# mrazomej/BarBay.jl

Measured on AMD Instinct MI355X. Metric: ELBO-grad steps/sec, 50k barcodes x 8 timepoints, higher is better.
Workload: dtype f64

## Files before the change

barbay.jl_amd/csrc/bb_engine.hip:

```cpp
#include "../../include/barbay_hip.h"
#include "bb_block.h"
#include "bb_persist.h"
#include "bb_resident.h"
#include "bb_stream.h"
#include "bb_inst.h"
#include "bb_hier.h"
#include "bb_ppc.h"
#include "bb_freq.h"
#include "bb_score.h"
#include "bb_chain.h"
#include "bb_logp.h"
#include "bb_mathprobe.h"

#include <algorithm>
#include <cmath>
#include <cstdarg>
#include <cstdio>
#include <cstdlib>
#include <cstring>
#include <ctime>
#include <string>
#include <type_traits>
#include <vector>

static thread_local char g_err[512] = "";
static int bb_fail(int code, const char* fmt, ...) {
    va_list ap;
    va_start(ap, fmt);
    vsnprintf(g_err, sizeof g_err, fmt, ap);
    va_end(ap);
    return code;
}
extern "C" const char* bb_last_error(void) { return g_err; }

#include "bb_backend.h"

extern "C" const char* bb_version(void) { return BB_BACKEND_VERSION; }

#define BB_ENTER(h) DevGuard bb_dev_guard_((h)->o.device)

struct BBTuning {
    bool no_hist_pack, no_host_tables, no_res, no_persist, no_stream, force_stream, any_parity, force_allreduce, p2p_self;
    bool no_graph, graph_collective, no_regroup, no_reorder, nb_set, lead_set;
    int nb, res_nb, ng, lead, nthr, row_l2;
};

static BBTuning read_tuning() {
    auto set = [](const char* n) { return getenv(n) != nullptr; };
    auto num = [](const char* n, int unset) { const char* v = getenv(n); return v ? atoi(v) : unset; };
    auto on = [&](const char* n) { return num(n, 0) > 0; };
    BBTuning t{};
    t.no_hist_pack = on("BB_NO_HIST_PACK");
    t.no_host_tables = on("BB_NO_HOST_TABLES");
    t.no_res = on("BB_NO_RES");
    t.no_persist = on("BB_NO_PERSIST");
    t.no_stream = on("BB_NO_STREAM");
    t.force_stream = on("BB_TUNE_STREAM");
    t.any_parity = on("BB_TUNE_AP");
    t.force_allreduce = on("BB_FORCE_ALLREDUCE");
    t.p2p_self = on("BB_P2P_SELF");
    t.no_graph = set("BB_NO_GRAPH");
    t.graph_collective = set("BB_GRAPH_COLLECTIVE");
    t.no_regroup = set("BB_NO_REGROUP");
    t.no_reorder = set("BB_NO_REORDER");
    t.nb_set = set("BB_TUNE_NB");
    t.nb = num("BB_TUNE_NB", 0);
    t.res_nb = num("BB_TUNE_RES_NB", 0);
    t.ng = num("BB_TUNE_NG", 0);
    t.lead_set = set("BB_TUNE_LEAD");
    t.lead = num("BB_TUNE_LEAD", 65);
    if (t.lead < 10 || t.lead > 100) t.lead = 100;
    t.nthr = num("BB_TUNE_NTHR", 0) >= 64 ? num("BB_TUNE_NTHR", 0) / 64 * 64 : 0;
    t.row_l2 = num("BB_TUNE_ROW_L2", 1) == 0 ? 0 : 1;
    return t;
}

enum { IMPL_TWO_KERNEL = 0, IMPL_PERSIST = 1, IMPL_RES = 2, IMPL_STREAM = 3 };
struct LaunchPlan {
    int impl = IMPL_TWO_KERNEL;
    int P = 0;
    int NB = 0, NBL = 0, nblk = 0;
    int ng = 8, pf = 0;
    bool ms = false;
    const void* fn = nullptr;
    std::string name;
    const char* why = nullptr;
};

struct DevBuf {
    double* p = nullptr;
    size_t cap = 0;
    int grow(size_t n) {
        if (cap >= n) return 0;
        if (p) dfree(p);
        p = nullptr;
        cap = 0;
        void* q = nullptr;
        int rc = dmalloc(&q, n * 8);
        if (!rc) { p = (double*)q; cap = n; }
        return rc;
    }
};
enum {
    BUF_EPS,
    BUF_DBG,
    BUF_BANDS,
    BUF_LOGP,
    BUF_CHAIN,
    BUF_COUNT
};

struct bb_handle {
    DevModel M{};
    DevState S{};
    bb_advi_opts o{};
    std::vector<bb_block_range> blocks;
    std::vector<void*> owned;
    long long dev_bytes = 0;
    int NB = 0, nthr = 0, nblk = 0, ngeno_blk = 0;
    int tile_cap = 0;
    size_t lds_doubles = 0;
    size_t lds_doubles_p0 = 0;
    size_t lds_doubles_p = 0;
    long long b_lo = 0, b_hi = 0;
    int cus = 256;
    int g_lo = 0, g_hi = 0;
    std::vector<int> geno_ptr_h;
    long long* d_tile_b = nullptr;
    int* d_tile_g = nullptr;
    long long step = 0;
    int sample = 0;
    double elbo_const = 0.0;
    std::vector<double> ld_omega, ld_zero;
    void* p2p_inbox = nullptr;
    size_t p2p_rows_bytes = 0, p2p_bytes = 0, p2p_gran_off = 0;
    double* d_segtab = nullptr;
    int* d_ldstab = nullptr;
    size_t segtab_cap = 0, ldstab_cap = 0;
    void* p2p_peer[BB_MAX_WORLD] = {};
    bool p2p_ready = false, p2p_on = false;
    unsigned p2p_seq = 0;
    unsigned epoch0 = 0;
    long long req_steps = 0;
    bool p2p_first = false;
    unsigned* hstatus = nullptr;
    double* bak_mu = nullptr;
    double* bak_om = nullptr;
    DevBuf buf[BUF_COUNT];
    std::vector<double> logp_host;
    bbStream stream{};
    double last_run_ms = 0, avg_sample_ms = 0, avg_update_ms = 0;
    int launches_last_run = 0;
    int graph_launches = 0;
    int64_t bytes_sample = 0, bytes_update = 0;
    BackendState be;
    BBTuning tune{};
    LaunchPlan plan;
    BRLay Yh{};
    BRLay* dY = nullptr;
    DevModel* dM = nullptr;
    DevState* dS = nullptr;
    BBLds* dL = nullptr;
    BBLds Lp{};
    std::vector<bb_handle*> shards;
    bool group_resident = false;
    double* theta_buf = nullptr;
    bool theta_stale = false;
    bool in_group = false;
    std::vector<long long> cidx;
    std::vector<int> perm_m;
    bool use_reduce() const { return o.world_size > 1 || M.kind == BB_MODEL_GENOTYPE || tune.force_allreduce; }
};

template <class T>
static int dalloc(bb_handle* h, T** p, size_t count) {
    void* q = nullptr;
    int rc = dmalloc(&q, count * sizeof(T));
    if (rc) return rc;
    h->owned.push_back(q);
    h->dev_bytes += (long long)(count * sizeof(T));
    *p = (T*)q;
    return dzero(q, count * sizeof(T), h->stream);
}

extern "C" void bb_default_opts(bb_advi_opts* o) {
    memset(o, 0, sizeof *o);
    o->samples_per_step = 1;
    o->optimizer = BB_OPT_TRUNCATED_ADAGRAD;
    o->eta = 0.1;
    o->tau = 40.0;
    o->window = 100;
    o->resum_every = 0;
    o->pre = 1.0;
    o->post = 0.9;
    o->seed = 0;
    o->device = 0;
    o->rank = 0;
    o->world_size = 1;
    o->steps_per_graph = 0;
    o->elbo_every = 0;
    o->n_devices = 1;
    o->device_ids = nullptr;
}

static void add_block(bb_handle* h, const char* name, int kind, long long n, long long* off) {
    bb_block_range b;
    memset(&b, 0, sizeof b);
    snprintf(b.name, sizeof b.name, "%s", name);
    b.lo = *off;
    b.hi = *off + n;
    h->blocks.push_back(b);
    h->M.blk_lo[kind] = b.lo;
    h->M.blk_hi[kind] = b.hi;
    *off += n;
}

static int upload_prior(bb_handle* h, int kind, const bb_prior* p, double dmean, double dstd, const char* name,
                        bool vector_only, double* sum_log_std) {
    const long long n = h->M.blk_hi[kind] - h->M.blk_lo[kind];
    DevPrior& dp = h->M.pri[kind];
    dp.mean_e = nullptr;
    dp.inv_var_e = nullptr;
    if (!p || !p->mean || !p->std || p->n == 0) {
        dp.mean = dmean;
        dp.inv_var = 1.0 / (dstd * dstd);
        *sum_log_std += (double)n * log(dstd);
        return 0;
    }
    if (p->n == 1 || (n == 1 && p->n == 1)) {
        if (!(p->std[0] > 0)) return bb_fail(BB_ERR_INVALID, "%s: std must be > 0", name);
        dp.mean = p->mean[0];
        dp.inv_var = 1.0 / (p->std[0] * p->std[0]);
        *sum_log_std += (double)n * log(p->std[0]);
        return 0;
    }
    if (vector_only) return bb_fail(BB_ERR_INVALID, "%s accepts only the Vector form [mean, std]", name);
    if (p->n != n) return bb_fail(BB_ERR_INVALID, "%s: Matrix form needs %lld rows, got %lld", name, n, (long long)p->n);
    std::vector<double> iv((size_t)n);
    for (long long i = 0; i < n; ++i) {
        if (!(p->std[i] > 0)) return bb_fail(BB_ERR_INVALID, "%s: std[%lld] must be > 0", name, i);
        iv[(size_t)i] = 1.0 / (p->std[i] * p->std[i]);
        *sum_log_std += log(p->std[i]);
    }
    double *dm = nullptr, *di = nullptr;
    int rc;
    if ((rc = dalloc(h, &dm, (size_t)n))) return rc;
    if ((rc = dalloc(h, &di, (size_t)n))) return rc;
    if ((rc = h2d(dm, p->mean, (size_t)n * 8, h->stream))) return rc;
    if ((rc = h2d(di, iv.data(), (size_t)n * 8, h->stream))) return rc;
    dp.mean = 0;
    dp.inv_var = 0;
    dp.mean_e = dm;
    dp.inv_var_e = di;
    return 0;
}

struct CreateCtx { BBTuning tune; bool loglambda_first; };
static int group_create(const bb_model_desc* md, const bb_advi_opts* opts, const CreateCtx& cx, bb_handle** out);
static void hist_rows(bb_handle* h) {
    DevModel& M = h->M;
    M.Dh = M.Dp;
    for (int k = 0; k < BK_COUNT; ++k) M.hd0[k] = M.hd1[k] = 0;
    for (int r = 0; r < BB_MAX_REP; ++r) M.hdl[r] = 0;
    if (h->o.world_size <= 1 || h->tune.no_hist_pack || M.Dp >= (1ll << 31)) return;
    const long long b0 = h->b_lo, nbt = h->b_hi - h->b_lo;
    const long long m0 = std::max(h->b_lo, M.nn) - M.nn, nmt = (std::max(h->b_hi, M.nn) - M.nn) - m0;
    long long c = 0;
    auto place = [&](long long a, long long len) { const long long at = c + ((a - c) & 1); c = at + len + 2; return a - at; };
    auto place_r = [&](int blk, long long a0, long long stride, long long len, int R) {
        const long long lp = len + 2 + ((stride - (len + 2)) & 1);
        const long long at = c + ((a0 - c) & 1);
        M.hd0[blk] = a0 - at;
        M.hd1[blk] = stride - lp;
        c = at + (long long)R * lp;
    };
    M.hd0[BK_SPOP] = place(M.blk_lo[BK_SPOP], M.blk_hi[BK_SPOP] - M.blk_lo[BK_SPOP]);
    M.hd0[BK_LSPOP] = place(M.blk_lo[BK_LSPOP], M.blk_hi[BK_LSPOP] - M.blk_lo[BK_LSPOP]);
    if (M.kind == BB_MODEL_FITNESS || M.kind == BB_MODEL_MULTIENV) {
        M.hd0[BK_S] = place(M.blk_lo[BK_S] + m0 * M.E, nmt * M.E);
        M.hd0[BK_LS] = place(M.blk_lo[BK_LS] + m0 * M.E, nmt * M.E);
    } else if (M.kind == BB_MODEL_GENOTYPE) {
        M.hd0[BK_S] = place(M.blk_lo[BK_S], M.G);
        M.hd0[BK_TT] = place(M.blk_lo[BK_TT] + m0, nmt);
        M.hd0[BK_LT] = place(M.blk_lo[BK_LT] + m0, nmt);
        M.hd0[BK_LS] = place(M.blk_lo[BK_LS] + m0, nmt);
    } else {
        const long long E_ = M.kind == BB_MODEL_MULTIENV_REPLICATE ? M.E : 1;
        M.hd0[BK_S] = place(M.blk_lo[BK_S] + m0 * E_, nmt * E_);
        for (int blk : {BK_TT, BK_LT, BK_LS}) place_r(blk, M.blk_lo[blk] + m0 * E_, M.nb * E_, nmt * E_, M.R);
    }
    for (int r = 0; r < M.R; ++r) M.hdl[r] = place(M.off_l[r] + b0 * M.T[r], nbt * M.T[r]);
    const long long Dh = (c + 7) & ~7ll;
    if (Dh >= M.Dp) {
        for (int k = 0; k < BK_COUNT; ++k) M.hd0[k] = M.hd1[k] = 0;
        for (int r = 0; r < BB_MAX_REP; ++r) M.hdl[r] = 0;
        return;
    }
    M.Dh = Dh;
}

static int create_inner(const bb_model_desc* md, const bb_advi_opts* opts, const CreateCtx& cx, bb_handle** out);
static int ensure_scratch(bb_handle* h);
static void owned_ranges(const bb_handle* sh, std::vector<std::pair<long long, long long>>& out);
static RunArgs make_args(const bb_handle* h, long long step, int sample, int S, bool apply, bool with_elbo);
static int theta_sync_local(bb_handle* const* hs, int n);
static int launch_persistent(bb_handle* h, long long nsteps);
static int run_enqueue(bb_handle* h, int64_t n_steps);
static int run_finish(bb_handle* h);

template <class F>
static void by_kind(int kind, F&& f) {
    switch (kind) {
    case 0: f(std::integral_constant<int, 0>{}); break;
    case 1: f(std::integral_constant<int, 1>{}); break;
    case 2: f(std::integral_constant<int, 2>{}); break;
    case 3: f(std::integral_constant<int, 3>{}); break;
    default: f(std::integral_constant<int, 4>{});
    }
}

static int uniform_T(const DevModel& M) {
    for (int r = 1; r < M.R; ++r) if (M.T[r] != M.T[0]) return 0;
    return M.T[0];
}

#ifndef BB_EMU
static bb_persist_kernel persist_kernel(int kind, int P, int nthr, bool xg = false, const char** nm = nullptr) {
#ifdef BB_FAST_BUILD
    if (nm) *nm = "(experiment build)";
    if (!xg && nthr > 512 && P == 1 && kind == 0) return k_persist<0, 1, 1024>;
    return nullptr;
#else
    return bb_persist_instance(kind, P, nthr, xg, nm);
#endif
}
static bb_res_kernel res_kernel(int kind, int P, int nthr, bool xg, int T, bool ap, bool ms = false, const char** nm = nullptr) {
#ifdef BB_FAST_BUILD
    if (nm) *nm = "(experiment build)";
    if (xg || ms) return nullptr;
    if (ap) {
        if (nthr > 512 && P == 1 && kind == 0) return k_res<0, 1, 1024, false, 0, true>;
        if (nthr > 256 && nthr <= 512 && P == 3 && kind == 3) return k_res<3, 3, 512, false, 0, true>;
        return nullptr;
    }
    if (nthr > 512 && P == 1 && kind == 0) return T == 8 ? k_res<0, 1, 1024, false, 8> : k_res<0, 1, 1024, false>;
    if (nthr > 512 && P == 1 && kind == 1) return T == 6 ? k_res<1, 1, 1024, false, 6> : k_res<1, 1, 1024, false>;
    if (nthr > 256 && nthr <= 512 && P == 2 && kind == 0) return T == 8 ? k_res<0, 2, 512, false, 8> : k_res<0, 2, 512, false>;
    if (nthr > 256 && nthr <= 512 && P == 3 && kind == 3) return T == 6 ? k_res<3, 3, 512, false, 6> : k_res<3, 3, 512, false>;
    if (nthr > 256 && nthr <= 512 && P == 2 && kind == 3) return T == 6 ? k_res<3, 2, 512, false, 6> : k_res<3, 2, 512, false>;
    if (nthr > 512 && P == 1 && kind == 2) return T == 8 ? k_res<2, 1, 1024, false, 8> : k_res<2, 1, 1024, false>;
    return nullptr;
#else
    switch (kind) {
    case 0: return bb_res_instance_k0(P, nthr, xg, T, ap, ms, nm);
    case 1: return bb_res_instance_k1(P, nthr, xg, T, ap, ms, nm);
    case 2: return bb_res_instance_k2(P, nthr, xg, T, ap, ms, nm);
    case 3: return bb_res_instance_k3(P, nthr, xg, T, ap, ms, nm);
    default: return bb_res_instance_k4(P, nthr, xg, T, ap, ms, nm);
    }
#endif
}
static bb_stream_kernel stream_kernel(int kind, int nthr, int T, const char** nm = nullptr, bool ms = false) {
#ifdef BB_FAST_BUILD
    if (nm) *nm = "(experiment build)";
    if (ms) return nullptr;
    if (nthr == 1024 && kind == 0 && T == 8) return k_stream<0, 1024, 8>;
    if (nthr == 1024 && kind == 2 && T == 8) return k_stream<2, 1024, 8>;
    if (nthr == 1024 && kind == 3 && T == 6) return k_stream<3, 1024, 6>;
    return nullptr;
#else
    return ms ? bb_stream_instance_ms(kind, nthr, T, nm) : bb_stream_instance(kind, nthr, T, nm);
#endif
}
static const void* resident_instance(const bb_handle* h, bool stream, int P, bool ms, std::string& name) {
    const char* nm = "";
    const void* k = stream ? (const void*)stream_kernel(h->M.kind, h->nthr, uniform_T(h->M), &nm, ms)
// ... 667 lines not shown
                double s = 0.0;
                for (long long b = 0; b < nb_; ++b)
                    s += log((double)md->counts[co + b * T + t + 1] + 0.5) - log((double)md->counts[co + b * T + t] + 0.5);
                piv[(size_t)(M.tcum[r] + t)] = s / (double)nb_;
            }
            co += (long long)T * M.B;
        }
    }
    {
        double* d = nullptr;
        BB_TRY(dalloc(h, &d, (size_t)M.Ttot));
        BB_TRY(h2d(d, piv.data(), (size_t)M.Ttot * 8, h->stream));
        M.piv = d;
    }

    if (has_env) {
        int* d = nullptr;
        BB_TRY(dalloc(h, &d, (size_t)M.Ttot));
        BB_TRY(h2d(d, md->env_idx, (size_t)M.Ttot * 4, h->stream));
        M.env_idx = d;
    }
    if (md->kind == BB_MODEL_GENOTYPE) {
        int *d = nullptr, *dp = nullptr, *dm = nullptr;
        BB_TRY(dalloc(h, &d, (size_t)M.nb));
        BB_TRY(h2d(d, md->geno_idx, (size_t)M.nb * 4, h->stream));
        M.geno_idx = d;
        std::vector<int> ptr((size_t)M.G + 1, 0), mem((size_t)M.nb);
        for (long long m = 0; m < M.nb; ++m) ptr[(size_t)md->geno_idx[m] + 1]++;
        for (int g = 0; g < M.G; ++g) ptr[(size_t)g + 1] += ptr[(size_t)g];
        std::vector<int> fill(ptr.begin(), ptr.end() - 1);
        for (long long m = 0; m < M.nb; ++m) mem[(size_t)fill[(size_t)md->geno_idx[m]]++] = (int)m;
        BB_TRY(dalloc(h, &dp, (size_t)M.G + 1));
        BB_TRY(dalloc(h, &dm, (size_t)M.nb));
        BB_TRY(h2d(dp, ptr.data(), ((size_t)M.G + 1) * 4, h->stream));
        BB_TRY(h2d(dm, mem.data(), (size_t)M.nb * 4, h->stream));
        M.geno_ptr = dp;
        M.geno_mem = dm;
        M.geno_sorted = 1;
        for (long long m = 1; m < M.nb; ++m) if (md->geno_idx[m] < md->geno_idx[m - 1]) { M.geno_sorted = 0; break; }
        h->geno_ptr_h = ptr;
    }

    double sum_log_std = 0.0;
    BB_TRY(upload_prior(h, BK_SPOP, &md->s_pop_prior, 0.0, 2.0, "s_pop_prior", false, &sum_log_std));
    BB_TRY(upload_prior(h, BK_LSPOP, &md->logsigma_pop_prior, 0.0, 1.0, "logsigma_pop_prior", false, &sum_log_std));
    BB_TRY(upload_prior(h, BK_S, &md->s_bc_prior, 0.0, 2.0, "s_bc_prior", false, &sum_log_std));
    BB_TRY(upload_prior(h, BK_LS, &md->logsigma_bc_prior, 0.0, 1.0, "logsigma_bc_prior", false, &sum_log_std));
    BB_TRY(upload_prior(h, BK_L, &md->loglambda_prior, 3.0, 3.0, "loglambda_prior", false, &sum_log_std));
    if (M.kind >= BB_MODEL_GENOTYPE) {
        BB_TRY(upload_prior(h, BK_TT, nullptr, 0.0, 1.0, "theta_tilde", true, &sum_log_std));
        BB_TRY(upload_prior(h, BK_LT, &md->logtau_prior, -2.0, 1.0, "logtau_prior", true, &sum_log_std));
    }
    {
        double nlik = 0.0;
        for (int r = 0; r < M.R; ++r) nlik += (double)(M.T[r] - 1) * (double)M.B;
        h->elbo_const = -sum_log_std - 0.5 * BB_LOG2PI * (double)M.D - sum_lgamma - 0.5 * BB_LOG2PI * nlik +
                        0.5 * (double)M.D * (1.0 + BB_LOG2PI);
    }

    h->b_lo = M.B * opts->rank / opts->world_size;
    h->b_hi = M.B * (opts->rank + 1) / opts->world_size;
    h->g_lo = 0;
    h->g_hi = M.G;
    if (M.kind == BB_MODEL_GENOTYPE && M.geno_sorted && opts->world_size > 1) {
        auto snap = [&](long long b, int* g) {
            if (b <= 0) { *g = 0; return (long long)0; }
            if (b >= M.B) { *g = M.G; return M.B; }
            if (b <= M.nn) { *g = 0; return b; }
            const int gg = md->geno_idx[b - M.nn];
            *g = gg;
            return M.nn + (long long)h->geno_ptr_h[(size_t)gg];
        };
        h->b_lo = snap(h->b_lo, &h->g_lo);
        h->b_hi = snap(h->b_hi, &h->g_hi);
        if (h->b_lo <= M.nn) h->g_lo = 0;
    }
    {
        int maxT = 0;
        for (int r = 0; r < M.R; ++r) maxT = std::max(maxT, M.T[r]);
        h->cus = dev_cus(opts->device, h->cus);
        const long long nbar = std::max<long long>(h->b_hi - h->b_lo, 1);
        int NB = (int)std::max<long long>((nbar + h->cus - 1) / h->cus, 32);
        if (h->tune.nb > 0) NB = h->tune.nb;
        const size_t lds_cap = (size_t)160 * 1024;
        int nthr = 0;
        for (;;) {
            const long long pairs = tile_pairs_bound(M, NB);
            nthr = pairs > 2048 ? 1024 : (pairs > 1024 ? 512 : (pairs > 512 ? 1024 : (pairs > 256 ? 512 : 256)));
            if (h->tune.nthr) nthr = h->tune.nthr;
            while (nthr < maxT) nthr <<= 1;
            const size_t need = (size_t)bb_lds_layout(M.R, M.E, M.kind, M.Ttot, M.nt1, M.K, NB, nthr).total * 8;
            if ((need <= lds_cap && (long long)NB * maxT < 65536) || NB <= 8) break;
            NB = (NB + 1) / 2;
        }
        const size_t need = (size_t)bb_lds_layout(M.R, M.E, M.kind, M.Ttot, M.nt1, M.K, NB, nthr).total * 8;
        if (need > 160 * 1024 || nthr > 1024 || (long long)NB * maxT >= 65536) {
            bb_destroy(h);
            return bb_fail(BB_ERR_UNSUPPORTED, "a tile of %d barcodes needs %zu bytes of LDS / %d threads (n_time or n_rep too large for this build)", NB, need, nthr);
        }
        h->NB = NB;
        h->nthr = nthr;
        h->lds_doubles = need / 8;
        h->lds_doubles_p0 = h->lds_doubles_p = (size_t)bb_lds_layout(M.R, M.E, M.kind, M.Ttot, M.nt1, M.K, NB, nthr, 1).total;
        h->nblk = (int)((nbar + NB - 1) / NB);
        h->tile_cap = h->nblk + 8;
        h->ngeno_blk = M.G > 0 ? (int)std::min<long long>(((M.G + 1) / 2 + 255) / 256, 64) : 0;
    }

    DevState& S = h->S;
    const size_t D = (size_t)M.D;
    BB_TRY(dalloc(h, &S.mu, D + 2));
    BB_TRY(dalloc(h, &S.om, D + 2));
    BB_TRY(dalloc(h, &S.acc_mu, D + 2));
    BB_TRY(dalloc(h, &S.acc_om, D + 2));
    BB_TRY(dalloc(h, &S.accl, 2 * D + 8));
    {
        double* oc = nullptr;
        const double v[8] = {opts->eta, opts->tau, opts->pre, opts->post, 0, 0, 0, 0};
        BB_TRY(dalloc(h, &oc, 8));
        BB_TRY(h2d(oc, v, sizeof v, h->stream));
        S.optc = oc;
    }
    hist_rows(h);
    if (opts->optimizer == BB_OPT_TRUNCATED_ADAGRAD) BB_TRY(dalloc(h, &S.hist, (size_t)opts->window * 2 * (size_t)M.Dh + 8));
    BB_TRY(dalloc(h, &S.partials, (size_t)M.K * (size_t)h->nblk));
    BB_TRY(dalloc(h, &S.totals, (size_t)M.K));
    BB_TRY(dalloc(h, &S.zg, (size_t)2 * M.nt1));
    BB_TRY(dalloc(h, &S.gbar, (size_t)32 * 10));
    BB_TRY(hostmap_alloc(&h->hstatus, &S.hstatus, 16));
    BB_TRY(dalloc(h, &S.prow, (size_t)h->tile_cap * (M.K + 2 * M.nt1)));
    BB_TRY(dalloc(h, &S.xrow, (size_t)2 * BB_NG_MAX * (M.K + 2 * M.nt1)));
    BB_TRY(dalloc(h, &S.grow, (size_t)(h->tile_cap + 16 * BB_NG_MAX) * bb_row_stride(M.K + 2 * M.nt1)));
    BB_TRY(dalloc(h, &S.gxrow, (size_t)2 * BB_NG_MAX * (M.K + 2 * M.nt1)));
    BB_TRY(dalloc(h, &S.rdy, (size_t)32 * (h->tile_cap + 2 * BB_NG_MAX)));
    BB_TRY(dalloc(h, &S.xtab, (size_t)BB_NG_MAX));
    BB_TRY(dalloc(h, &S.xsel, (size_t)h->tile_cap));
    BB_TRY(dalloc(h, &S.ztheta, (size_t)std::max(M.G, 1)));
    BB_TRY(dalloc(h, &S.gsum, (size_t)std::max(M.G, 1)));
    BB_TRY(dalloc(h, &S.ds, (size_t)M.nb));
    BB_TRY(dalloc(h, &S.geno_el, (size_t)std::max(h->ngeno_blk, 1)));
    BB_TRY(dalloc(h, &S.elbo_ring, (size_t)BB_ELBO_RING));
    BB_TRY(dalloc(h, &S.elbo_sample, (size_t)opts->samples_per_step + 64));
    BB_TRY(dalloc(h, &S.ctr, (size_t)2));
    BB_TRY(dalloc(h, &S.stamps, (size_t)h->tile_cap * (32 + 64)));
    S.eps_in = nullptr;

    {
        const long long nb_sh = h->b_hi - h->b_lo;
        double frac = (double)nb_sh / (double)M.B;
        const double Dsh = (double)M.D * frac;
        const double cnts = 4.0 * (double)cnt * frac;
        h->bytes_sample = (int64_t)(16.0 * Dsh + cnts);
        const double optb = opts->optimizer == BB_OPT_TRUNCATED_ADAGRAD ? 64.0 : 32.0;
        h->bytes_update = (int64_t)((16.0 + 16.0 + optb) * Dsh + cnts);
    }
    BB_TRY(setup_persistent(h, h->o.launch_mode));
    BB_TRY(sync_descriptors(h));
    BB_TRY(bb_init_meanfield(h));
    *out = h;
    return BB_OK;
}


static void perm_gather(const bb_handle* h, const double* caller, double* internal) {
    const size_t D = h->cidx.size();
    for (size_t i = 0; i < D; ++i) internal[i] = caller[(size_t)h->cidx[i]];
}
static void perm_scatter(const bb_handle* h, const double* internal, double* caller) {
    const size_t D = h->cidx.size();
    for (size_t i = 0; i < D; ++i) caller[(size_t)h->cidx[i]] = internal[i];
}

extern "C" int bb_create(const bb_model_desc* md, const bb_advi_opts* opts, bb_handle** out) {
    if (!md || !opts || !out) return bb_fail(BB_ERR_INVALID, "null argument");
    const bool geno_ok = md->kind == BB_MODEL_GENOTYPE && md->geno_idx && md->n_bc > 1 && md->n_geno >= 1 && md->n_neutral >= 1 && md->n_time &&
                         md->counts && md->n_rep == 1 && md->n_time[0] >= 2 && md->n_time[0] <= 255;
    CreateCtx cx{read_tuning(), false};
    bool regroup = geno_ok && !cx.tune.no_regroup;
    if (regroup) {
        bool sorted = true, valid = true;
        for (long long m = 0; m < md->n_bc && valid; ++m) {
            if (md->geno_idx[m] < 0 || md->geno_idx[m] >= md->n_geno) valid = false;
            else if (m > 0 && md->geno_idx[m] < md->geno_idx[m - 1]) sorted = false;
        }
        regroup = valid && !sorted;
    }
    cx.loglambda_first = geno_ok && !(md->n_time[0] & 1) && ((md->n_geno + md->n_bc) & 1) && !cx.tune.no_reorder;
    if (!regroup && !cx.loglambda_first) return create_inner(md, opts, cx, out);
    const long long nn = md->n_neutral, nb = md->n_bc, B = nn + nb;
    const int T = md->n_time[0];
    std::vector<int> perm((size_t)nb);
    for (long long m = 0; m < nb; ++m) perm[(size_t)m] = (int)m;
    if (regroup) std::stable_sort(perm.begin(), perm.end(), [&](int a, int b) { return md->geno_idx[a] < md->geno_idx[b]; });
    auto src = [&](long long b) { return b < nn ? b : nn + perm[(size_t)(b - nn)]; };
    bb_model_desc md2 = *md;
    std::vector<int64_t> counts2;
    std::vector<int32_t> geno2;
    std::vector<double> lsm, lss, llm, lls;
    if (regroup) {
        counts2.resize((size_t)B * T);
        for (long long b = 0; b < B; ++b) memcpy(&counts2[(size_t)b * T], md->counts + src(b) * T, (size_t)T * sizeof(int64_t));
        geno2.resize((size_t)nb);
        for (long long m = 0; m < nb; ++m) geno2[(size_t)m] = md->geno_idx[perm[(size_t)m]];
        md2.counts = counts2.data();
        md2.geno_idx = geno2.data();
        if (md->logsigma_bc_prior.mean && md->logsigma_bc_prior.std && md->logsigma_bc_prior.n == nb && nb > 1) {
            lsm.resize((size_t)nb); lss.resize((size_t)nb);
            for (long long m = 0; m < nb; ++m) { lsm[(size_t)m] = md->logsigma_bc_prior.mean[perm[(size_t)m]]; lss[(size_t)m] = md->logsigma_bc_prior.std[perm[(size_t)m]]; }
            md2.logsigma_bc_prior.mean = lsm.data(); md2.logsigma_bc_prior.std = lss.data();
        }
        if (md->loglambda_prior.mean && md->loglambda_prior.std && md->loglambda_prior.n == (int64_t)B * T && B * T > 1) {
            llm.resize((size_t)B * T); lls.resize((size_t)B * T);
            for (long long b = 0; b < B; ++b)
                for (int t = 0; t < T; ++t) { llm[(size_t)b * T + t] = md->loglambda_prior.mean[src(b) * T + t]; lls[(size_t)b * T + t] = md->loglambda_prior.std[src(b) * T + t]; }
            md2.loglambda_prior.mean = llm.data(); md2.loglambda_prior.std = lls.data();
        }
    }
    int rc = create_inner(&md2, opts, cx, out);
    if (rc) return rc;
    bb_handle* h = *out;
    const DevModel& M = h->M;
    if (regroup) h->perm_m = perm;
    const int order[BK_COUNT] = {BK_SPOP, BK_LSPOP, BK_S, BK_TT, BK_LT, BK_LS, BK_L};
    long long clo[BK_COUNT] = {0};
    {
        std::vector<bb_block_range> cb;
        long long off = 0;
        for (int k : order) {
            bb_block_range b;
            memset(&b, 0, sizeof b);
            for (const bb_block_range& ib : h->blocks) if (ib.lo == M.blk_lo[k] && ib.hi == M.blk_hi[k] && ib.hi > ib.lo) snprintf(b.name, sizeof b.name, "%s", ib.name);
            clo[k] = off;
            b.lo = off;
            b.hi = off + (M.blk_hi[k] - M.blk_lo[k]);
            off = b.hi;
            cb.push_back(b);
        }
        h->blocks = cb;
    }
    h->cidx.resize((size_t)M.D);
    for (int k : order)
        for (long long j = 0; j < M.blk_hi[k] - M.blk_lo[k]; ++j) h->cidx[(size_t)(M.blk_lo[k] + j)] = clo[k] + j;
    if (regroup) {
        for (int k : {BK_TT, BK_LT, BK_LS})
            for (long long m = 0; m < nb; ++m) h->cidx[(size_t)(M.blk_lo[k] + m)] = clo[k] + perm[(size_t)m];
        for (long long b = nn; b < B; ++b)
            for (int t = 0; t < T; ++t) h->cidx[(size_t)(M.blk_lo[BK_L] + b * T + t)] = clo[BK_L] + src(b) * T + t;
    }
    return BB_OK;
}

extern "C" int bb_get_owned(bb_handle* h, int64_t* idx, int64_t* n) {
    if (!h || !idx || !n) return bb_fail(BB_ERR_INVALID, "null argument");
    std::vector<std::pair<long long, long long>> rg;
    if (h->shards.empty()) owned_ranges(h, rg);
    else for (bb_handle* sh : h->shards) owned_ranges(sh, rg);
    int64_t c = 0;
    for (auto& r : rg)
        for (long long i = r.first; i < r.second; ++i) idx[c++] = h->cidx.empty() ? i : h->cidx[(size_t)i];
    *n = c;
    return BB_OK;
}

extern "C" int bb_get_permutation(bb_handle* h, int64_t* caller_index) {
    if (!h || !caller_index) return bb_fail(BB_ERR_INVALID, "null argument");
    for (long long i = 0; i < h->M.D; ++i) caller_index[i] = h->cidx.empty() ? i : h->cidx[(size_t)i];
    return BB_OK;
}

static void p2p_release(bb_handle* h);
static void group_destroy(bb_handle* g);
extern "C" void bb_destroy(bb_handle* h) {
    if (!h) return;
    if (!h->shards.empty()) { group_destroy(h); return; }
    BB_ENTER(h);
    stream_quiesce(h->stream, h->be);
    p2p_release(h);
    hostmap_free(h->hstatus);
    for (void* p : h->owned) dfree(p);
    for (DevBuf& b : h->buf) if (b.p) dfree(b.p);
    stream_close(h->stream);
    delete h;
}

extern "C" int64_t bb_num_latents(const bb_handle* h) { return h ? h->M.D : 0; }

extern "C" int bb_get_layout(const bb_handle* h, bb_block_range* blocks, int32_t* n) {
    if (!h || !blocks || !n) return bb_fail(BB_ERR_INVALID, "null argument");
    *n = (int32_t)h->blocks.size();
    for (size_t i = 0; i < h->blocks.size(); ++i) blocks[i] = h->blocks[i];
    return BB_OK;
}

static RunArgs make_args(const bb_handle* h, long long step, int sample, int S, bool apply, bool with_elbo) {
    RunArgs A;
    memset(&A, 0, sizeof A);
    A.b_lo = h->b_lo;
    A.b_hi = h->b_hi;
    A.rank = h->o.rank;
    A.world = h->o.world_size;
    A.xepoch0 = h->epoch0;
    A.spin_limit = 1u << 23;
    A.row_l2 = h->tune.row_l2;
    A.nblk = h->nblk;
    A.nblk_alloc = h->tile_cap - 8;
    A.ng = 8;
    A.par = (int)(step & 1);
    A.sample = sample;
    A.S = S;
    A.first_sample = sample == 0;
    A.last_sample = sample == S - 1;
    A.apply = apply ? 1 : 0;
    A.with_elbo = with_elbo ? 1 : 0;
    A.count_globals = h->o.rank == 0;
    A.opt = h->o.optimizer;
    A.W = h->o.window;
    A.resum_every = h->o.resum_every;
    A.elbo_every = h->o.elbo_every;
    A.eta = h->o.eta;
    A.tau = h->o.tau;
    A.pre = h->o.pre;
    A.post = h->o.post;
    A.seed = h->o.seed;
    A.elbo_const = h->elbo_const;
    if (h->use_reduce()) { A.red = h->S.totals; A.nred = 1; }
    else { A.red = h->S.partials; A.nred = h->nblk; }
    return A;
}

static int ensure_scratch(bb_handle* h) {
    if (h->S.zsv) return BB_OK;
    const size_t D = (size_t)h->M.D, n = (D + 2 + 1) & ~(size_t)1;
    double* slab = nullptr;
    int rc = dalloc(h, &slab, 7 * n);
    if (rc) return rc;
    h->S.zsv = slab; h->S.asv = slab + n; h->S.hsv = slab + 2 * n; h->S.gacc_mu = slab + 3 * n; h->S.gacc_om = slab + 4 * n;
    h->bak_mu = slab + 5 * n; h->bak_om = slab + 6 * n;
    return h->dS ? h2d(h->dS, &h->S, sizeof(DevState), h->stream) : BB_OK;
}

static int launch_sample(bb_handle* h, const RunArgs& A) {
    if (!h->S.zsv) return bb_fail(BB_ERR_DEVICE, "internal: the two-kernel step's scratch arrays were not allocated (ensure_scratch)");
    int rc = 0;
    by_kind(h->M.kind, [&](auto kindc) {
        rc = launch(h->stream, k_sample<decltype(kindc)::value>, h->nblk, h->nthr, h->lds_doubles, desc_ptr(h->dM, &h->M), desc_ptr(h->dS, &h->S), A, h->NB);
    });
    return rc;
}
static int launch_update(bb_handle* h, const RunArgs& A) {
    if (!h->S.zsv) return bb_fail(BB_ERR_DEVICE, "internal: the two-kernel step's scratch arrays were not allocated (ensure_scratch)");
    int rc = 0;
    by_kind(h->M.kind, [&](auto kindc) {
        rc = launch(h->stream, k_update<decltype(kindc)::value>, h->nblk, h->nthr, h->lds_doubles, desc_ptr(h->dM, &h->M), desc_ptr(h->dS, &h->S), A, h->NB);
    });
    return rc;
}
static int launch_reduce(bb_handle* h) {
    return launch(h->stream, k_reduce, 1, 256, (size_t)16 * h->M.K, h->M, h->S, h->nblk, h->ngeno_blk);
}
static int launch_geno(bb_handle* h, const RunArgs& A, int do_update, int do_sample, int upd_par) {
    if (!h->S.zsv) return bb_fail(BB_ERR_DEVICE, "internal: the two-kernel step's scratch arrays were not allocated (ensure_scratch)");
    return launch(h->stream, k_geno, h->ngeno_blk, 256, 256 + 64, h->M, h->S, A, do_update, do_sample, upd_par);
}
static int launch_geno_sum(bb_handle* h) {
    const long long m_lo = std::max(h->b_lo, h->M.nn) - h->M.nn, m_hi = std::max(h->b_hi, h->M.nn) - h->M.nn;
    const int gsb = (int)std::min<long long>((h->M.G + 31) / 32, 1024);
    return launch(h->stream, k_geno_sum, gsb, 256, 256, h->M, h->S, m_lo, m_hi);
}

static int allreduce(bb_handle* h, double* buf, size_t n) {
    if (h->o.world_size == 1 && !h->tune.force_allreduce) return 0;
    return comm_allreduce(h->be, h->stream, buf, n, h->o.world_size);
}

static size_t theta_rows(const bb_handle* h) { return 6 + (h->o.optimizer == BB_OPT_TRUNCATED_ADAGRAD ? 2 * (size_t)h->o.window : 0); }
static bool theta_partial(const bb_handle* h) { return h->M.kind == BB_MODEL_GENOTYPE && (h->g_lo > 0 || h->g_hi < h->M.G); }
static int theta_pack(bb_handle* h, int unpack) {
    const size_t n = theta_rows(h) * (size_t)h->M.G;
    int rc;
    if (!h->theta_buf && (rc = dalloc(h, &h->theta_buf, n))) return rc;
    const int W = h->o.optimizer == BB_OPT_TRUNCATED_ADAGRAD ? h->o.window : 0;
    const int nb = (int)std::min<size_t>((n + 255) / 256, 512);
    return launch(h->stream, k_theta_pack, nb, 256, 0, h->M, h->S, h->theta_buf, h->g_lo, h->g_hi, W, unpack);
}
static int theta_sync_comm(bb_handle* h) {
    int rc;
    if ((rc = theta_pack(h, 0))) return rc;
    if ((rc = allreduce(h, h->theta_buf, theta_rows(h) * (size_t)h->M.G))) return rc;
    if ((rc = theta_pack(h, 1))) return rc;
    h->theta_stale = false;
    return dsync(h->stream);
}
static int theta_sync_local(bb_handle* const* hs, int n) {
    if (n < 2 || !theta_partial(hs[0])) return 0;
    const size_t len = theta_rows(hs[0]) * (size_t)hs[0]->M.G;
    std::vector<double> part(len), total(len, 0.0);
    int rc;
    for (int i = 0; i < n; ++i) {
        BB_ENTER(hs[i]);
        if ((rc = theta_pack(hs[i], 0)) || (rc = d2h(part.data(), hs[i]->theta_buf, len * 8, hs[i]->stream))) return rc;
        for (size_t k = 0; k < len; ++k) total[k] += part[k];
    }
    for (int i = 0; i < n; ++i) {
        BB_ENTER(hs[i]);
        if ((rc = h2d(hs[i]->theta_buf, total.data(), len * 8, hs[i]->stream)) || (rc = theta_pack(hs[i], 1)) || (rc = dsync(hs[i]->stream))) return rc;
        hs[i]->theta_stale = false;
    }
    return 0;
}

static int sample_half(bb_handle* h, const RunArgs& A) {
    int rc;
    if (h->M.kind == BB_MODEL_GENOTYPE && (rc = launch_geno(h, A, 0, 1, 0))) return rc;
    if ((rc = launch_sample(h, A))) return rc;
    if (h->use_reduce() && (rc = launch_reduce(h))) return rc;
    return 0;
}
static int update_half(bb_handle* h, const RunArgs& A) {
    int rc;
    if ((rc = launch_update(h, A))) return rc;
    if (h->M.kind == BB_MODEL_GENOTYPE) {
        if ((rc = launch_geno_sum(h))) return rc;
        if ((rc = allreduce(h, h->S.gsum, (size_t)h->M.G))) return rc;
        if ((rc = launch_geno(h, A, 1, 0, A.par))) return rc;
    }
    return 0;
}

static bool elbo_wanted(const bb_handle* h, long long step) {
    return h->o.elbo_every > 0 && step % h->o.elbo_every == 0;
}

static int enqueue_step(bb_handle* h, long long step) {
    const int S = h->o.samples_per_step;
    int rc;
    for (int s = 0; s < S; ++s) {
        RunArgs A = make_args(h, step, s, S, true, elbo_wanted(h, step));
        if ((rc = sample_half(h, A))) return rc;
        if ((rc = allreduce(h, h->S.totals, (size_t)h->M.K))) return rc;
        if ((rc = update_half(h, A))) return rc;
    }
    return 0;
}

static int set_step(bb_handle* h, long long step) {
    unsigned long long c[2] = {(unsigned long long)step, (unsigned long long)step};
    h->step = step;
    h->sample = 0;
    return h2d(h->S.ctr, c, sizeof c, h->stream);
}

static int reset_optimizer(bb_handle* h) {
    const size_t D = (size_t)h->M.D;
    int rc;
    if ((rc = dzero(h->S.accl, (2 * D + 8) * 4, h->stream))) return rc;
    if (h->o.optimizer == BB_OPT_TRUNCATED_ADAGRAD) {
        if ((rc = dzero(h->S.hist, (size_t)h->o.window * 2 * (size_t)h->M.Dh * 8, h->stream))) return rc;
        if ((rc = dzero(h->S.acc_mu, D * 8, h->stream))) return rc;
        if ((rc = dzero(h->S.acc_om, D * 8, h->stream))) return rc;
    } else {
        std::vector<double> a(D, 1e-8);
        if ((rc = h2d(h->S.acc_mu, a.data(), D * 8, h->stream))) return rc;
        if ((rc = h2d(h->S.acc_om, a.data(), D * 8, h->stream))) return rc;
    }
    std::vector<double> nanv(BB_ELBO_RING, NAN);
    if ((rc = h2d(h->S.elbo_ring, nanv.data(), nanv.size() * 8, h->stream))) return rc;
    h->epoch0 += (unsigned)h->req_steps + 1u;
    h->req_steps = 0;
    return set_step(h, 0);
}


static int p2p_alloc_inbox(bb_handle* h);
static int p2p_wire(bb_handle* h, void* const* bases);
static int p2p_probe_launch(bb_handle* h, unsigned** res);
static int p2p_probe_collect(bb_handle* h, unsigned* res, int32_t* ok);
static void owned_ranges(const bb_handle* sh, std::vector<std::pair<long long, long long>>& out) {
    const DevModel& M = sh->M;
    const long long b_lo = sh->b_lo, b_hi = sh->b_hi;
    const long long m_lo = std::max(b_lo, M.nn) - M.nn, m_hi = std::max(b_hi, M.nn) - M.nn;
    for (int r = 0; r < M.R; ++r) out.push_back({M.off_l[r] + b_lo * M.T[r], M.off_l[r] + b_hi * M.T[r]});
    if (M.kind == BB_MODEL_GENOTYPE && sh->g_hi > sh->g_lo) out.push_back({M.blk_lo[BK_S] + sh->g_lo, M.blk_lo[BK_S] + sh->g_hi});
    if (m_hi <= m_lo) return;
    if (M.kind == BB_MODEL_FITNESS || M.kind == BB_MODEL_MULTIENV) {
        out.push_back({M.blk_lo[BK_S] + m_lo * M.E, M.blk_lo[BK_S] + m_hi * M.E});
        out.push_back({M.blk_lo[BK_LS] + m_lo * M.E, M.blk_lo[BK_LS] + m_hi * M.E});
    } else if (M.kind == BB_MODEL_GENOTYPE) {
        for (int k : {BK_TT, BK_LT, BK_LS}) out.push_back({M.blk_lo[k] + m_lo, M.blk_lo[k] + m_hi});
    } else {
        const long long E_ = M.kind == BB_MODEL_MULTIENV_REPLICATE ? M.E : 1;
        out.push_back({M.blk_lo[BK_S] + m_lo * E_, M.blk_lo[BK_S] + m_hi * E_});
        for (int r = 0; r < M.R; ++r)
            for (int k : {BK_TT, BK_LT, BK_LS}) out.push_back({M.blk_lo[k] + (r * M.nb + m_lo) * E_, M.blk_lo[k] + (r * M.nb + m_hi) * E_});
    }
}

static void group_destroy(bb_handle* g) {
    for (bb_handle* sh : g->shards) bb_destroy(sh);
    g->shards.clear();
    delete g;
}

static int group_create(const bb_model_desc* md, const bb_advi_opts* opts, const CreateCtx& cx, bb_handle** out) {
    const int n = opts->n_devices;
    if (n > BB_MAX_WORLD) return bb_fail(BB_ERR_UNSUPPORTED, "at most %d devices per handle", BB_MAX_WORLD);
    if (opts->world_size != 1 || opts->rank != 0) return bb_fail(BB_ERR_INVALID, "n_devices > 1 needs rank 0 / world_size 1 (the handle shards by itself)");
    bb_handle* g = new bb_handle();
    g->o = *opts;
    g->o.device = opts->device_ids ? opts->device_ids[0] : 0;
    g->tune = cx.tune;
    int rc = 0;
    for (int i = 0; i < n && !rc; ++i) {
        bb_advi_opts o = *opts;
        o.n_devices = 1;
        o.device_ids = nullptr;
        o.device = opts->device_ids ? opts->device_ids[i] : i;
        o.rank = i;
        o.world_size = n;
        o.launch_mode = opts->launch_mode == 1 ? 1 : 0;
        bb_handle* sh = nullptr;
        rc = create_inner(md, &o, cx, &sh);
        if (!rc) { sh->in_group = true; g->shards.push_back(sh); }
        if (!rc && memcmp(sh->M.blk_lo, g->shards[0]->M.blk_lo, sizeof sh->M.blk_lo))
            rc = bb_fail(BB_ERR_INVALID, "shard %d lays the latents out differently from shard 0", i);
    }
    if (rc) { group_destroy(g); return rc; }
    g->M = g->shards[0]->M;
    g->blocks = g->shards[0]->blocks;
    g->b_lo = 0;
    g->b_hi = g->M.B;
    bool ok = opts->launch_mode != 1;
    for (int i = 0; i < n && ok; ++i)
        for (int j = 0; j < n && ok; ++j) {
            const int di = g->shards[i]->o.device, dj = g->shards[j]->o.device;
            if (di != dj && !peer_enable(di, dj)) ok = false;
        }
    void* bases[BB_MAX_WORLD] = {};
    for (int i = 0; i < n && ok; ++i) {
        BB_ENTER(g->shards[i]);
        ok = p2p_alloc_inbox(g->shards[i]) == BB_OK;
        bases[i] = g->shards[i]->p2p_inbox;
    }
    for (int i = 0; i < n && ok; ++i) { BB_ENTER(g->shards[i]); ok = p2p_wire(g->shards[i], bases) == BB_OK; }
    if (ok) {
        unsigned* res[BB_MAX_WORLD] = {};
        for (int i = 0; i < n; ++i) { BB_ENTER(g->shards[i]); if (p2p_probe_launch(g->shards[i], &res[i]) != BB_OK) ok = false; }
        for (int i = 0; i < n; ++i) {
            BB_ENTER(g->shards[i]);
            int32_t good = 0;
            if (p2p_probe_collect(g->shards[i], res[i], &good) != BB_OK || !good) ok = false;
        }
    }
    if (ok) for (int i = 0; i < n && ok; ++i) ok = bb_p2p_enable(g->shards[i], 1) == BB_OK;
    if (ok) for (int i = 1; i < n && ok; ++i) ok = (g->shards[i]->plan.impl >= IMPL_RES) == (g->shards[0]->plan.impl >= IMPL_RES);
    if (!ok) for (bb_handle* sh : g->shards) if (sh->p2p_ready) (void)bb_p2p_enable(sh, 0);
    g->group_resident = ok;
    if (!ok && opts->launch_mode == 2) {
        const std::string why(g_err);
        group_destroy(g);
        return bb_fail(BB_ERR_UNSUPPORTED, "launch_mode = 2: the shards cannot run resident launches with peer-mapped inboxes: %s", why.c_str());
    }
    *out = g;
    return BB_OK;
}

static int group_run(bb_handle* g, int64_t n_steps) {
    int rc = 0;
    if (g->group_resident) {
        rc = group_run_resident(g, n_steps);
    } else {
        const int S = g->o.samples_per_step < 1 ? 1 : g->o.samples_per_step;
        const size_t K = (size_t)g->shards[0]->M.K, G = (size_t)g->shards[0]->M.G;
        const bool geno = g->shards[0]->M.kind == BB_MODEL_GENOTYPE;
        std::vector<double> part(std::max(K, G)), total(std::max(K, G));
        for (bb_handle* sh : g->shards) { BB_ENTER(sh); if ((rc = ensure_scratch(sh))) return rc; }
        auto exchange = [&](size_t n, double* DevState::*buf) -> int {
            std::fill(total.begin(), total.begin() + n, 0.0);
            for (bb_handle* sh : g->shards) {
                BB_ENTER(sh);
                int r = d2h(part.data(), sh->S.*buf, n * 8, sh->stream);
                if (r) return r;
                for (size_t k = 0; k < n; ++k) total[k] += part[k];
            }
            for (bb_handle* sh : g->shards) { BB_ENTER(sh); int r = h2d(sh->S.*buf, total.data(), n * 8, sh->stream); if (r) return r; }
            return 0;
        };
        for (int64_t it = 0; it < n_steps && !rc; ++it) {
            for (int smp = 0; smp < S && !rc; ++smp) {
                std::vector<RunArgs> As;
                for (bb_handle* sh : g->shards) As.push_back(make_args(sh, sh->step, smp, S, true, elbo_wanted(sh, sh->step)));
                for (size_t i = 0; i < g->shards.size() && !rc; ++i) { BB_ENTER(g->shards[i]); rc = sample_half(g->shards[i], As[i]); }
                if (!rc) rc = exchange(K, &DevState::totals);
                for (size_t i = 0; i < g->shards.size() && !rc; ++i) {
                    BB_ENTER(g->shards[i]);
                    rc = launch_update(g->shards[i], As[i]);
                    if (!rc && geno) rc = launch_geno_sum(g->shards[i]);
                }
                if (!rc && geno) rc = exchange(G, &DevState::gsum);
                for (size_t i = 0; i < g->shards.size() && !rc && geno; ++i) { BB_ENTER(g->shards[i]); rc = launch_geno(g->shards[i], As[i], 1, 0, As[i].par); }
            }
            for (bb_handle* sh : g->shards) sh->step++;
        }
        for (bb_handle* sh : g->shards) { BB_ENTER(sh); const int r = dsync(sh->stream); if (r && !rc) rc = r; }
    }
    g->step = g->shards[0]->step;
    return rc;
// ... 585 lines not shown
```

barbay.jl_amd/csrc/bb_resident.h:

```cpp
#pragma once
#include "bb_persist.h"

#define BR_NCV 12
#if defined(BB_EMU) || defined(BR_NO_FENCE)
#define BR_SCHED_FENCE() ((void)0)
#else
#define BR_SCHED_FENCE() __builtin_amdgcn_sched_barrier(0)
#endif
#define BR_MAXT 16

struct BRSeg { long long lo, hi; int tbeg, span, blk, kind, ldsoff, r, lpb, T; double pm, iv; const double* mean_e; const double* iv_e; long long blo; int rstride, pad; };
#define BR_SEG_DOUBLES 12

struct BRLay {
    BBLds L;
    int zl, NBT;
    int zr0[BB_MAX_REP];
    int zlw, stw;
    int st[6], SU, nst;
    int eps;
    int hbuf;
    int racc;
    int racc_r[BB_MAX_REP], rw[BB_MAX_REP];
    int rowmap;
    int iG, csum;
    int rtab;
    int ftab;
    int envt;
    int gas;
    int gix;
    int seg;
    int total;
    int lpb[BB_MAX_REP];
};

#define BR_ST(Y, i) ((Y).st[0] + (i) * (Y).stw)
static inline int br_lpb(int T) { return (T + 1) / 2; }
BB_HD int br_lpb_stream(int T) { const int l = (T + 1) / 2; return l <= 1 ? 1 : (l <= 2 ? 2 : (l <= 4 ? 4 : 8)); }

static inline long long br_tile_span(const DevModel& M, long long NB, bool globals, bool stream = false) {
    long long p = 0;
    for (int r = 0; r < M.R; ++r) p = ((p + 63) & ~63ll) + NB * (stream ? br_lpb_stream(M.T[r]) : br_lpb(M.T[r]));
    if (M.kind == 0 || M.kind == 1) p += 2 * (NB * M.E / 2 + 1);
    else if (M.kind == 2) p += 4 * (NB / 2 + 1);
    else if (M.kind == 3) p += (NB / 2 + 1) + 3ll * M.R * (NB / 2 + 1);
    else p += (NB * M.E / 2 + 1) + 3ll * M.R * (NB * M.E / 2 + 1);
    if (globals) p += 2 * (M.nt1 / 2 + 1);
    return p;
}

static inline bool br_eligible(const DevModel& M) {
    if (M.kind == 2 && !M.geno_sorted) return false;
    if (M.quirk || M.Ttot > 64) return false;
    for (int r = 0; r < M.R; ++r) if (M.T[r] < 2 || M.T[r] > BR_MAXT) return false;
    return true;
}
static inline bool br_any_parity(const DevModel& M) {
    if (M.blk_lo[BK_L] & 1) return true;
    for (int r = 0; r < M.R; ++r) if ((M.T[r] & 1) || (M.off_l[r] & 1)) return true;
    return false;
}

struct BRHdr { int rowmap, tmap, wk, zgl, Lt, invS, cc, wbar, gglob, misc, part, Dt, elbt, iG, csum, ftab, rtab, envt, seg, end; };
#ifndef BB_EMU
__host__ __device__
#endif
inline constexpr BRHdr br_header(int K, int nt1, int Ttot, int R) {
    BRHdr h{};
    const int KK = K + 2 * nt1;
    int o = 0;
    h.rowmap = o;  o += K + 1;
    h.tmap = o;    o += (K + 1) / 2 + 1;
    h.wk = o;      o += KK;
    h.zgl = o;     o += 2 * nt1;
    h.Lt = o;      o += Ttot;
    h.invS = o;    o += Ttot;
    h.cc = o;      o += Ttot + 1;
    h.wbar = o;    o += Ttot + 1;
    h.gglob = o;   o += 2 * nt1;
    h.misc = o;    o += 16 + BB_MAX_REP;
    h.part = o;    o += 32;
    h.Dt = o;      o += Ttot + 1;
    h.elbt = o;    o += Ttot;
    h.iG = o;      o += Ttot;
    h.csum = o;    o += BB_MAX_REP;
    o = (o + 1) & ~1;
    h.ftab = o;    o += 2 * Ttot;
    h.rtab = o;    o += 2 * R;
    h.envt = o;    o += (Ttot + 1) / 2 + 1;
    o = (o + 1) & ~1;
    h.seg = o;     o += BR_SEG_DOUBLES * (4 + 4 * R + 1);
    h.end = (o + 1) & ~1;
    return h;
}

static inline
#ifndef BB_EMU
__host__ __device__
#endif
BRLay br_layout(const DevModel& M, int NB, int NT, int P, int xg_rows, bool own_hbuf = false, bool stream = false) {
    BRLay Y;
    const int X = (M.kind == 1) ? M.E : (M.kind == 4 ? M.E * M.R : M.R);
    const int KK = M.K + 2 * M.nt1;
    int o = 0;
    int lmax = 1;
    for (int r = 0; r < BB_MAX_REP; ++r) { Y.lpb[r] = r < M.R ? (stream ? br_lpb_stream(M.T[r]) : br_lpb(M.T[r])) : 1; if (Y.lpb[r] > lmax) lmax = Y.lpb[r]; }
    BBLds& L = Y.L;
    L = BBLds{};
    Y.NBT = 0;
    for (int r = 0; r < BB_MAX_REP; ++r) { Y.zr0[r] = Y.NBT; if (r < M.R) Y.NBT += NB * (M.T[r] + 1); }
    Y.NBT = (Y.NBT + 1) & ~1;
    if (stream) { long long sp = 0; for (int r = 0; r < M.R; ++r) sp += (long long)NB * (M.T[r] / 2); Y.NBT = (int)(2 * sp + 2); }
    {
        const BRHdr H = br_header(M.K, M.nt1, M.Ttot, M.R);
        Y.rowmap = H.rowmap; L.tmap = H.tmap; L.wk = H.wk; L.zgl = H.zgl; L.Lt = H.Lt; L.invS = H.invS; L.cc = H.cc; L.GG = H.wbar; L.wbar = H.wbar;
        L.gglob = H.gglob; L.misc = H.misc; L.part = H.part; L.Dt = H.Dt; L.elbt = H.elbt; Y.iG = H.iG; Y.csum = H.csum; Y.ftab = H.ftab;
        Y.rtab = H.rtab; Y.envt = H.envt; Y.seg = H.seg; L.seg = H.seg;
        o = H.end;
    }
    Y.zlw = stream ? 1 : 2;
    Y.zl = o;      o += Y.zlw * Y.NBT;
    Y.SU = NB * X;
    Y.nst = stream ? (M.kind <= 1 ? 2 : 4) : (M.kind <= 1 ? 3 : 6);
    Y.stw = 2 * Y.SU;
    for (int i = 0; i < 6; ++i) { Y.st[i] = o; if (i < Y.nst) o += Y.stw; }
    o = (o + 1) & ~1;
    Y.gas = o;     o += stream ? (M.kind >= 2 ? Y.SU : 0) : ((M.kind == 2 || M.kind == 3) ? 2 * Y.SU : 0);
    Y.gix = o;     o += M.kind == 2 ? Y.SU + 1 : 0;
    o = (o + 1) & ~1;
    o = (o + 1) & ~1;
    Y.racc = o;
    int racc_total = 0;
    for (int r = 0; r < BB_MAX_REP; ++r) {
        Y.racc_r[r] = Y.racc + racc_total;
        Y.rw[r] = r < M.R ? (stream ? (NT / (M.R == 1 ? 16 : 64)) * Y.lpb[r] : (int)(((long long)NB * Y.lpb[r] + 63) & ~63ll)) : 0;
        if (r < M.R) racc_total += BR_NCV * (Y.rw[r] + 4);
    }
    int busy;
    if (stream) {
        Y.hbuf = Y.racc;
        busy = racc_total > 2 * Y.SU ? racc_total : 2 * Y.SU;
        o += busy;
        Y.eps = o;     o += NT / 2;
    } else if (own_hbuf) {
        Y.eps = Y.racc;
        busy = 2 * P * NT;
        o += racc_total > busy ? racc_total : busy;
        o = (o + 1) & ~1;
        Y.hbuf = o;    o += 4 * P * NT;
    } else {
        Y.hbuf = Y.racc;
        Y.eps = Y.hbuf + 4 * P * NT;
        busy = 6 * P * NT;
        o += racc_total > busy ? racc_total : busy;
    }
    { const int nch = xg_rows / 8 > 5 ? xg_rows / 8 : 5;
      L.red = o;     o += 2 * 128 + nch * ((KK + 63) & ~63) + 16; }
    (void)lmax;
    L.total = Y.total = (o + 1) & ~1;
    return Y;
}

template <int P>
struct BRSt {
    bb_d2 mu[P], om[P], am[P], ao[P];
    bb_d2 a[P], h[P];
    bb_d2 z[P];
    bb_d2 lam[P];
    long long i0[P];
    int meta[P];
    int zoff[P];
    int uo[P][3];
    int pt[P];
    int rb[P];
    int thoff[P];
    unsigned cnt[P][2];
    bb_f4 lo[P];
    bb_d2 gp[P];
    bb_d2 gm[P], go[P];
    double el;
};

enum { BRM_A0 = 1 << 4, BRM_A1 = 1 << 5, BRM_VALID = 1 << 6, BRM_MUT = 1 << 7, BRM_PREV = 1 << 8, BRM_NEXT = 1 << 9 };

template <bool AP> BB_DEV bool br_pair_aligned(long long i0) { return !AP || !(i0 & 1); }
template <bool AP> BB_DEV bb_d2 br_load_pair(const double* base, long long i0, bool a0, bool a1) {
    if (a0 && a1 && br_pair_aligned<AP>(i0)) return *(const bb_d2*)(base + i0);
    return bb_d2{a0 ? base[i0] : 0.0, a1 ? base[i0 + 1] : 0.0};
}
template <bool AP> BB_DEV void br_store_pair_stream(double* base, long long i0, bool a0, bool a1, bb_d2 v) {
#ifndef BB_EMU
    if (a0 && a1 && br_pair_aligned<AP>(i0)) {
        typedef double bb_v2d __attribute__((ext_vector_type(2)));
        bb_v2d w = {v.x, v.y};
        __builtin_nontemporal_store(w, (bb_v2d*)(base + i0));
        return;
    }
    if (a0) __builtin_nontemporal_store(v.x, base + i0);
    if (a1) __builtin_nontemporal_store(v.y, base + i0 + 1);
#else
    if (a0 && a1 && br_pair_aligned<AP>(i0)) { *(bb_d2*)(base + i0) = v; return; }
    if (a0) base[i0] = v.x;
    if (a1) base[i0 + 1] = v.y;
#endif
}
template <bool AP> BB_DEV void br_store_pair(double* base, long long i0, bool a0, bool a1, bb_d2 v) {
    if (a0 && a1 && br_pair_aligned<AP>(i0)) { *(bb_d2*)(base + i0) = v; return; }
    if (a0) base[i0] = v.x;
    if (a1) base[i0 + 1] = v.y;
}

BB_HD BBTile br_tile(const DevModel& M, const RunArgs& A, int block, int NB) {
    if (A.nbl <= 0) return bb_tile(M, A, block, NB);
    const int nlead = bbp_groups(A);
    BBTile t;
    t.NB = NB;
    const int cap = block < nlead ? A.nbl : NB;
    t.b0 = block < nlead ? A.b_lo + (long long)block * A.nbl : A.b_lo + (long long)nlead * A.nbl + (long long)(block - nlead) * NB;
    long long b1 = t.b0 + cap < A.b_hi ? t.b0 + cap : A.b_hi;
    if (t.b0 > A.b_hi) t.b0 = A.b_hi;
    t.nbt = (int)(b1 > t.b0 ? b1 - t.b0 : 0);
    long long ns = M.nn - t.b0;
    t.nshift = (int)(ns < 0 ? 0 : (ns > t.nbt ? t.nbt : ns));
    t.m0 = t.b0 + t.nshift - M.nn;
    t.nmt = t.nbt - t.nshift;
    return t;
}

BB_HD BBTile br_tile_geno(const DevModel& M, const DevState& S, int block, int NB) {
    BBTile t;
    t.NB = NB;
    t.b0 = S.tile_b[block];
    t.nbt = (int)(S.tile_b[block + 1] - t.b0);
    long long ns = M.nn - t.b0;
    t.nshift = (int)(ns < 0 ? 0 : (ns > t.nbt ? t.nbt : ns));
    t.m0 = t.b0 + t.nshift - M.nn;
    t.nmt = t.nbt - t.nshift;
    return t;
}

template <int KIND>
BB_HD int br_build_segs(BRSeg* sg, const DevModel& M, const BRLay& Y, const BBTile& t, bool globals, int g0 = 0, int g1 = 0) {
    int n = 0, cur = 0;
    auto add = [&](int blk, int kind, long long lo, long long cnt, int ldsoff, int r, int lpb, int T) {
        if (cnt <= 0) return;
        BRSeg s;
        s.lo = lo; s.hi = lo + cnt; s.blk = blk; s.kind = kind; s.ldsoff = ldsoff; s.r = r; s.lpb = lpb; s.T = T;
        s.rstride = kind == SK_L ? Y.rw[r] + 4 : 0; s.pad = (int)bb_hdelta(M, blk, r);
        s.pm = M.pri[blk].mean; s.iv = M.pri[blk].inv_var; s.mean_e = M.pri[blk].mean_e; s.iv_e = M.pri[blk].inv_var_e; s.blo = M.blk_lo[blk];
        if (kind == SK_L) { cur = (cur + 63) & ~63; s.span = (int)(cnt / T) * lpb; }
        else s.span = bb_seg_pairs(lo, lo + cnt);
        s.tbeg = cur;
        cur += s.span;
        sg[n++] = s;
    };
    for (int r = 0; r < M.R; ++r)
        add(BK_L, SK_L, M.off_l[r] + t.b0 * M.T[r], (long long)t.nbt * M.T[r], Y.zr0[r], r, Y.lpb[r], M.T[r]);
    if (KIND == 2) {
        add(BK_S, SK_TH_R, M.blk_lo[BK_S] + g0, g1 - g0, 0, 0, 0, 0);
        add(BK_TT, SK_TT_R, M.blk_lo[BK_TT] + t.m0, t.nmt, 0, 0, 0, M.T[0]);
        add(BK_LT, SK_LT_R, M.blk_lo[BK_LT] + t.m0, t.nmt, 0, 0, 0, M.T[0]);
        add(BK_LS, SK_LS_R, M.blk_lo[BK_LS] + t.m0, t.nmt, 0, 0, 0, M.T[0]);
    } else if (t.nmt > 0) {
        if (KIND == 0 || KIND == 1) {
            const int E = KIND == 1 ? M.E : 1;
            add(BK_S, SK_S, M.blk_lo[BK_S] + t.m0 * E, (long long)t.nmt * E, 0, 0, 0, M.T[0]);
            add(BK_LS, SK_LS_E, M.blk_lo[BK_LS] + t.m0 * E, (long long)t.nmt * E, 0, 0, 0, M.T[0]);
        } else {
            const int E_ = KIND == 4 ? M.E : 1;
            add(BK_S, SK_TH_R, M.blk_lo[BK_S] + t.m0 * E_, (long long)t.nmt * E_, 0, 0, 0, 0);
            for (int r = 0; r < M.R; ++r) {
                const long long o = ((long long)r * M.nb + t.m0) * E_;
                add(BK_TT, SK_TT_R, M.blk_lo[BK_TT] + o, (long long)t.nmt * E_, r * t.NB * E_, r, 0, M.T[r]);
                add(BK_LT, SK_LT_R, M.blk_lo[BK_LT] + o, (long long)t.nmt * E_, r * t.NB * E_, r, 0, M.T[r]);
                add(BK_LS, SK_LS_R, M.blk_lo[BK_LS] + o, (long long)t.nmt * E_, r * t.NB * E_, r, 0, M.T[r]);
            }
        }
    }
    if (globals) {
        add(BK_SPOP, SK_GS, M.blk_lo[BK_SPOP], M.blk_hi[BK_SPOP] - M.blk_lo[BK_SPOP], 0, 0, 0, 0);
        add(BK_LSPOP, SK_GLS, M.blk_lo[BK_LSPOP], M.blk_hi[BK_LSPOP] - M.blk_lo[BK_LSPOP], 0, 0, 0, 0);
    }
    sg[n].tbeg = cur;
    return n;
}

template <int KIND, int P, bool AP = false, int LPBC = 0, bool CNT = true>
BB_DEV void br_desc(const DevModel& M, const BRLay& Y, const BBTile& t, const BRSeg* sg, int nseg, int g0, int g1, int p, BRSt<P>& st, int k, const double* lds) {
    const int* gx = (const int*)(lds + Y.gix);
    const int* rtb = (const int*)(lds + Y.rtab);
    const int* envt = (const int*)(lds + Y.envt);
    const int E = (KIND == 1 || KIND == 4) ? M.E : 1;
    int si = -1;
    if (LPBC && nseg > 0 && p >= sg[0].tbeg && p < sg[0].tbeg + sg[0].span) si = 0;
    else for (int i = 0; i < nseg; ++i) if (p >= sg[i].tbeg && p < sg[i].tbeg + sg[i].span) si = i;
    int meta = 15;
    long long i0 = 0;
    st.zoff[k] = 0; st.uo[k][0] = st.uo[k][1] = st.uo[k][2] = 0; st.pt[k] = 0; st.cnt[k][0] = st.cnt[k][1] = 0u;
    st.rb[k] = 0; st.thoff[k] = 0;
    if (si >= 0) {
        const BRSeg s = sg[si];
        meta = s.kind | (si << 12);
        if (s.kind == SK_L) {
            const int q = p - s.tbeg, bl = LPBC ? q / LPBC : q / s.lpb, kk = q - bl * (LPBC ? LPBC : s.lpb);
            st.rb[k] = Y.racc_r[s.r] + q;
            if (2 * kk < s.T) {
                const int t0 = 2 * kk;
                i0 = s.lo + (long long)bl * s.T + t0;
                meta |= BRM_A0 | (t0 + 1 < s.T ? BRM_A1 : 0) | BRM_VALID | (t0 > 0 ? BRM_PREV : 0) | (t0 + 2 < s.T ? BRM_NEXT : 0);
                st.zoff[k] = s.ldsoff + bl * (s.T + 1) + t0;
                st.pt[k] = rtb[4 * s.r] + t0;
                if (bl >= t.nshift) {
                    meta |= BRM_MUT;
                    const int ml = bl - t.nshift;
                    const int base = KIND >= 3 ? (s.r * t.NB + ml) * E : ml * E;
                    st.thoff[k] = KIND >= 3 ? s.r * t.NB * E : (KIND == 2 ? ml - gx[ml] : 0);
                    for (int d = 0; d < 3; ++d) {
                        const int tt = t0 - 1 + d;
                        const int e = (E > 1 && tt >= 0 && tt < s.T - 1) ? envt[rtb[4 * s.r] + tt + 1] : 0;
                        st.uo[k][d] = base + e;
                    }
                }
                if (CNT) {
                    const int co = rtb[4 * s.r + 3];
                    const long long cb = (co >= 0 ? (long long)co : M.cnt_off[s.r]) + t.b0 * s.T + (long long)bl * s.T + t0;
                    st.cnt[k][0] = M.counts[cb];
                    st.cnt[k][1] = t0 + 1 < s.T ? M.counts[cb + 1] : 0u;
                }
            }
        } else {
            const int q = p - s.tbeg;
            i0 = 2 * ((s.lo >> 1) + q);
            const bool a0 = i0 >= s.lo, a1 = i0 + 1 < s.hi;
            meta |= (a0 ? BRM_A0 : 0) | (a1 ? BRM_A1 : 0) | BRM_VALID;
            st.zoff[k] = s.ldsoff + (int)(i0 - s.lo);
            st.thoff[k] = s.ldsoff;
            if (KIND == 2 && s.kind == SK_TH_R) {
                for (int x = 0; x < 2; ++x) {
                    const long long gl = (i0 - s.lo) + x;
                    int v = 0;
                    if (gl >= 0 && gl < g1 - g0) {
                        if (gl < Y.SU) v = gx[Y.SU + (int)gl];
                        else {
                            const long long g = g0 + gl;
                            const int n = M.geno_ptr[g + 1] - M.geno_ptr[g];
                            v = (n > 0 ? (int)(M.geno_mem[M.geno_ptr[g]] - t.m0) : 0) | (n << 16);
                        }
                    }
                    st.uo[k][x] = v;
                }
            } else if (s.kind < SK_GS) {
                int env = 0;
                for (int x = 0; x < 2; ++x) {
                    int j = (int)(i0 - s.lo) + x;
                    if (j < 0) j = 0;
                    const int ml = j / E, e = j - ml * E;
                    st.uo[k][x] = t.nshift + ml;
                    if (KIND == 2) env |= ((j < t.nmt ? gx[j] : 0) & 0xffff) << (16 * x);
                    else env |= e << (8 * x);
                }
                st.uo[k][2] = env;
                st.pt[k] = s.r;
            }
        }
    }
    st.i0[k] = i0;
    st.meta[k] = meta;
}

BB_HD void br_table_row(const DevModel& M, const BRLay& Y, int j, int* rm2, int* tmapj) {
    int code = 0, col = 0;
    for (int r = 0; r < M.R; ++r) {
        const int T = M.T[r], q0 = j - M.kq[r];
        if (q0 < 0 || q0 >= 6 * T - 5) continue;
        int tt, q;
        if (q0 < T) { tt = q0; q = 0; } else { tt = (q0 - T) / 5; q = 1 + (q0 - T) - 5 * tt; }
        code = Y.lpb[r] | (1 << 24);
        col = Y.racc_r[r] + ((tt & 1) * 6 + q) * (Y.rw[r] + 4) + (tt >> 1);
    }
    rm2[0] = code;
    rm2[1] = col;
    int tj = -1;
    for (int r = 0; r < M.R; ++r) { const int tt = j - M.kq[r]; if (tt >= 0 && tt < M.T[r]) tj = M.tcum[r] + tt; }
    *tmapj = tj;
}
BB_HD void br_table_time(const DevModel& M, const BBLds& L, int j, int* ft) {
    int r = 0;
    while (r + 1 < M.R && j >= M.tcum[r + 1]) ++r;
    const int tt = j - M.tcum[r], T = M.T[r];
    ft[0] = tt < T - 1 ? L.wk + M.kq[r] + T + 5 * tt : -1;
    ft[1] = M.off_t[r] + tt;
    ft[2] = tt > 0 ? 1 : 0;
    ft[3] = 0;
}
BB_HD void br_table_rep(const DevModel& M, const BRLay& Y, int r, int* rt) {
    rt[0] = M.tcum[r]; rt[1] = Y.zr0[r]; rt[2] = M.T[r];
    rt[3] = M.cnt_off[r] < (1ll << 31) ? (int)M.cnt_off[r] : -1;
}

template <int KIND>
BB_DEV void br_tile_setup(BBCtx& cx, const DevModel& M, const DevState& S, const RunArgs& A, const BRLay& Y, int NB, int ncol_or_neg) {
    double* lds = cx.lds;
    const BBLds& L = Y.L;
    const BBTile t = KIND == 2 ? br_tile_geno(M, S, cx.block, NB) : br_tile(M, A, cx.block, NB);
    const int g0 = KIND == 2 ? S.tile_g[cx.block] : 0, g1 = KIND == 2 ? S.tile_g[cx.block + 1] : 0;
    BRSeg* sg = (BRSeg*)(lds + Y.seg);
    int* li = (int*)(lds + L.misc);
    const int KK = M.K + 2 * M.nt1;
    BB_PASS(cx, tid) {
        if (S.segtab) {
            const double* src = S.segtab + (long long)cx.block * S.segtab_stride;
            const int nd = S.segtab_stride - 1;
            for (int i = tid; i < nd; i += cx.nthr) lds[Y.seg + i] = src[i];
            if (tid == 0) li[0] = ((const int*)(src + nd))[0];
        } else if (tid == 0) li[0] = br_build_segs<KIND>(sg, M, Y, t, cx.block == 0, g0, g1);
        if (tid == 0) { li[1] = bb_get_word(S.gbar + 1) == 0u ? 1 : 0; li[2] = ncol_or_neg < 0 ? t.nbt : ncol_or_neg; }
        if (tid == 0) {
            const int xcc = br_xcc_id(), NG = bbp_groups(A);
            li[4] = A.row_l2 ? 0 : -1; li[5] = xcc; li[6] = (int)A.launch_tag; li[7] = NG;
            S.xsel[cx.block] = li[4];
            if (cx.block < NG) bb_set_word64(S.xtab + cx.block, ((unsigned long long)A.launch_tag << 32) | (unsigned)xcc);
        }
        for (int k = tid; k < KK; k += cx.nthr) lds[L.wk + k] = 0.0;
        for (int i = tid; i < Y.zlw * Y.NBT; i += cx.nthr) lds[Y.zl + i] = 0.0;
        for (int i = tid; i < Y.nst * Y.stw; i += cx.nthr) lds[Y.st[0] + i] = 0.0;
        if (tid <= M.Ttot) { lds[L.cc + tid] = 0.0; lds[L.wbar + tid] = 0.0; lds[L.Dt + tid] = 0.0; }
        if (tid < M.Ttot) ((int*)(lds + Y.envt))[tid] = (KIND == 1 || KIND == 4) ? M.env_idx[tid] : 0;
        if (S.ldstab) { for (int i = tid; i < 4 * M.R; i += cx.nthr) ((int*)(lds + Y.rtab))[i] = S.ldstab[3 * M.K + 4 * M.Ttot + i]; }
        else for (int rr = tid; rr < M.R; rr += cx.nthr) br_table_rep(M, Y, rr, (int*)(lds + Y.rtab) + 4 * rr);
        if (KIND == 2) {
            int* gx = (int*)(lds + Y.gix);
            for (int j = tid; j < t.nmt; j += cx.nthr) gx[j] = M.geno_idx[t.m0 + j] - g0;
            for (int j = tid; j < g1 - g0 && j < Y.SU; j += cx.nthr) {
                const int g = g0 + j, n = M.geno_ptr[g + 1] - M.geno_ptr[g];
                gx[Y.SU + j] = (n > 0 ? (int)(M.geno_mem[M.geno_ptr[g]] - t.m0) : 0) | (n << 16);
            }
        }
    }
    BB_STAMP_RT(cx, S, 7);
    BB_SYNC(cx);
    BB_STAMP_RT(cx, S, 8);
    int* rm = (int*)(lds + Y.rowmap);
    if (S.ldstab) {
        const int K = M.K, Tt = M.Ttot, R = M.R;
        BB_PASS(cx, tid) {
            for (int i = tid; i < 2 * K; i += cx.nthr) rm[i] = S.ldstab[i];
            for (int i = tid; i < K; i += cx.nthr) ((int*)(lds + L.tmap))[i] = S.ldstab[2 * K + i];
            for (int i = tid; i < 4 * Tt; i += cx.nthr) ((int*)(lds + Y.ftab))[i] = S.ldstab[3 * K + i];
        }
    } else {
        BB_PASS(cx, tid) {
            for (int j = tid; j < M.K; j += cx.nthr) br_table_row(M, Y, j, rm + 2 * j, (int*)(lds + L.tmap) + j);
            for (int j = tid; j < M.Ttot; j += cx.nthr) br_table_time(M, L, j, (int*)(lds + Y.ftab) + 4 * j);
        }
    }
    BB_STAMP_RT(cx, S, 9);
}

template <int KIND, int P, bool AP = false>
BB_DEV void br_prologue(BBCtx& cx, const DevModel& M, const DevState& S, const RunArgs& A, const BRLay& Y, int NB, BRSt<P>* stv) {
    double* lds = cx.lds;
    const BBLds& L = Y.L;
    const BBTile t = KIND == 2 ? br_tile_geno(M, S, cx.block, NB) : br_tile(M, A, cx.block, NB);
    const int g0 = KIND == 2 ? S.tile_g[cx.block] : 0, g1 = KIND == 2 ? S.tile_g[cx.block + 1] : 0;
    const BRSeg* sg = (const BRSeg*)(lds + Y.seg);
    const int* li = (const int*)(lds + L.misc);
    br_tile_setup<KIND>(cx, M, S, A, Y, NB, -1);
    BB_PASS(cx, tid) {
        const int nseg = li[0];
        BRSt<P>& st = BB_PSTATE(stv, tid);
#pragma unroll
        for (int k = 0; k < P; ++k) {
            br_desc<KIND, P, AP>(M, Y, t, sg, nseg, g0, g1, tid + k * cx.nthr, st, k, lds);
            const long long i0 = st.i0[k];
            const int meta = st.meta[k];
            const bool a0 = meta & BRM_A0, a1 = meta & BRM_A1;
            st.mu[k] = br_load_pair<AP>(S.mu, i0, a0, a1);
            st.om[k] = br_load_pair<AP>(S.om, i0, a0, a1);
            st.am[k] = br_load_pair<AP>(S.acc_mu, i0, a0, a1);
            st.ao[k] = br_load_pair<AP>(S.acc_om, i0, a0, a1);
            st.lo[k] = bb_load_lo(S, i0, a0, a1);
            st.a[k] = st.h[k] = st.z[k] = st.lam[k] = st.gp[k] = bb_d2{0.0, 0.0};
        }
    }
    BB_STAMP_RT(cx, S, 10);
    BB_SYNC(cx);
}

template <int P> struct BRIdx { long long i0[P]; int meta[P]; };

template <int P, bool MAYODD>
#ifdef BB_EMU
static inline
#else
__device__ __attribute__((noinline))
#endif
void br_draw_call(bb_d2* eps, int nthr, int tid, unsigned long long seed, unsigned step, unsigned stream,
                  long long i0a, long long i0b, long long i0c, long long i0d, int ma, int mb, int mc, int md) {
    BRIdx<P> ix;
    { const long long i0v[4] = {i0a, i0b, i0c, i0d}; const int mv[4] = {ma, mb, mc, md};
#pragma unroll
      for (int k = 0; k < P; ++k) { ix.i0[k] = i0v[k]; ix.meta[k] = mv[k]; } }
#pragma unroll
    for (int k = 0; k < P; ++k) {
        if (!(ix.meta[k] & BRM_VALID)) continue;
        const bool odd = MAYODD && (ix.i0[k] & 1);
        double e0 = 0.0, e1 = 0.0;
#pragma nounroll
        for (int rep = 0; rep < (odd ? 2 : 1); ++rep) {
            double a, b;
            bb_normal_pair(seed, (unsigned long long)(ix.i0[k] >> 1) + (unsigned long long)rep, step, stream, &a, &b);
            if (rep == 0) { e0 = odd ? b : a; e1 = b; }
            else e1 = a;
        }
        eps[k * nthr + tid] = bb_d2{e0, e1};
    }
}

template <int KIND, int P, bool AP = false>
BB_DEV void br_draw_ahead(BBCtx& cx, const RunArgs& A, const BRLay& Y, BRSt<P>* stv, unsigned long long step, unsigned stream = 0u) {
    bb_d2* eps = (bb_d2*)(cx.lds + Y.eps);
    BB_PASS(cx, tid) {
        BRSt<P>& st = BB_PSTATE(stv, tid);
        static_assert(P <= 4, "br_draw_call takes four pair slots");
        br_draw_call<P, AP>(eps, cx.nthr, tid, A.seed, (unsigned)step, stream, st.i0[0], P > 1 ? st.i0[P > 1 ? 1 : 0] : 0, P > 2 ? st.i0[P > 2 ? 2 : 0] : 0,
                            P > 3 ? st.i0[P > 3 ? 3 : 0] : 0, st.meta[0], P > 1 ? st.meta[P > 1 ? 1 : 0] : 0, P > 2 ? st.meta[P > 2 ? 2 : 0] : 0, P > 3 ? st.meta[P > 3 ? 3 : 0] : 0);
    }
}

template <int KIND> BB_DEV int br_stage_raw(int kind) {
    if (KIND <= 1) return kind == SK_S ? 0 : 2;
    return kind == SK_TH_R ? 3 : (kind == SK_TT_R ? 0 : (kind == SK_LT_R ? 4 : 5));
}
template <int KIND> BB_DEV int br_stage_trn(int kind) {
    if (KIND <= 1) return kind == SK_LS_E ? 1 : -1;
    return kind == SK_LT_R ? 1 : (kind == SK_LS_R ? 2 : -1);
}
template <int KIND>
BB_DEV void br_unit_sw(const double* lds, const BRLay& Y, int buf, int o, int thoff, double* s, double* w) {
    const double* b = lds + buf * Y.SU;
    if (KIND <= 1) { *s = b[BR_ST(Y, 0) + o]; *w = b[BR_ST(Y, 1) + o]; }
    else { *s = fma(b[BR_ST(Y, 1) + o], b[BR_ST(Y, 0) + o], b[BR_ST(Y, 3) + o - thoff]); *w = b[BR_ST(Y, 2) + o]; }
}

#ifdef BB_EMU
#define BR_HDELTA(HD, lds, Y, meta) (((const BRSeg*)((lds) + (Y).seg))[(meta) >> 12].pad)
#else
#define BR_HDELTA(HD, lds, Y, meta) ((HD) ? ((const BRSeg*)((lds) + (Y).seg))[(meta) >> 12].pad : 0)
#endif
template <int P, bool HD = false>
BB_DEV void br_prefetch_slot(BBCtx& cx, const DevModel& M, const DevState& S, const RunArgs& A, const BRLay& Y, BRSt<P>* stv, int slot);
template <int KIND, int P> BB_DEV void br_pair_prior(const double* lds, const BRLay& Y, const BRSt<P>& st, int k, bool a0, bool a1, double* pm0, double* iv0, double* pm1, double* iv1);
template <int KIND, int P, bool MS = false, bool HD = false>
BB_DEV void br_sample(BBCtx& cx, const DevModel& M, const DevState& S, const RunArgs& A, const BRLay& Y, BRSt<P>* stv, int buf, int slot, bool prefetch = true, bool want_el = false) {
    double* lds = cx.lds;
    const BBLds& L = Y.L;
    BB_STAMP(cx, S, 20);
    BB_STAMP_WAVE(cx, S, A, 1);
    if (A.pf == 1 && prefetch) br_prefetch_slot<P, HD>(cx, M, S, A, Y, stv, slot);
    BB_PASS(cx, tid) {
        BRSt<P>& st = BB_PSTATE(stv, tid);
#pragma unroll
        for (int k = 0; k < P; ++k) {
#ifdef BB_EMU
            if (!(st.meta[k] & BRM_VALID)) continue;
#else
            if (P > 1 && __builtin_amdgcn_ballot_w64((st.meta[k] & BRM_VALID) != 0) == 0ull) continue;
#endif
            const bb_d2 e = ((const bb_d2*)(lds + Y.eps))[k * cx.nthr + tid];
            double sp0, sg0, sp1, sg1;
            bb_softplus_sigmoid(st.om[k].x, &sp0, &sg0);
            bb_softplus_sigmoid(st.om[k].y, &sp1, &sg1);
            st.z[k] = bb_d2{fma(sp0, e.x, st.mu[k].x), fma(sp1, e.y, st.mu[k].y)};
            st.a[k] = bb_d2{e.x * sg0, e.y * sg1};
            st.h[k] = bb_d2{sg0 * bb_rcp(sp0), sg1 * bb_rcp(sp1)};
            if (MS && want_el) {
                if (k == 0) st.el = 0.0;
                const int meta = st.meta[k], kd = meta & 15;
                const bool counted = (meta & BRM_VALID) && (kd < SK_GS || A.count_globals);
                if (counted) {
                    const bool a0 = meta & BRM_A0, a1 = meta & BRM_A1;
                    double pm0, iv0, pm1, iv1;
                    br_pair_prior<KIND>(lds, Y, st, k, a0, a1, &pm0, &iv0, &pm1, &iv1);
                    if (a0) st.el += -0.5 * (st.z[k].x - pm0) * (st.z[k].x - pm0) * iv0 + bb_log(sp0);
                    if (a1) st.el += -0.5 * (st.z[k].y - pm1) * (st.z[k].y - pm1) * iv1 + bb_log(sp1);
                }
            }
            BR_SCHED_FENCE();
            const int kd = st.meta[k] & 15;
            const double f = (kd == SK_LS_E || (KIND >= 2 && kd == SK_LS_R)) ? -2.0 : 1.0;
#ifndef BB_EMU
            if (__builtin_amdgcn_ballot_w64((st.meta[k] & BRM_VALID) && (kd == SK_L || (kd < SK_GS && br_stage_trn<KIND>(kd) >= 0))) == 0ull) st.lam[k] = bb_d2{0.0, 0.0};
            else
#endif
            st.lam[k] = bb_d2{bb_exp(f * st.z[k].x), bb_exp(f * st.z[k].y)};
            BR_SCHED_FENCE();
            if (MS && want_el && (st.meta[k] & BRM_VALID)) {
                const int meta = st.meta[k];
                if (kd == SK_L) {
                    st.el += (double)st.cnt[k][0] * st.z[k].x - st.lam[k].x;
                    if (meta & BRM_A1) st.el += (double)st.cnt[k][1] * st.z[k].y - st.lam[k].y;
                } else if (kd == SK_LS_E || (KIND >= 2 && kd == SK_LS_R)) {
                    const BRSeg* sgk = (const BRSeg*)(lds + Y.seg) + (meta >> 12);
                    const int T1 = sgk->T - 1;
#pragma unroll
                    for (int x = 0; x < 2; ++x) {
                        if (!(meta & (x ? BRM_A1 : BRM_A0))) continue;
                        int n = T1;
                        if (KIND == 1 || KIND == 4) {
                            const int* envt = (const int*)(lds + Y.envt);
                            const int e_ = (st.uo[k][2] >> (8 * x)) & 255, tc = KIND == 4 ? M.tcum[st.pt[k]] : 0;
                            n = 0;
                            for (int tt = 0; tt < T1; ++tt) n += envt[tc + tt + 1] == e_ ? 1 : 0;
                        }
                        st.el -= (x ? st.z[k].y : st.z[k].x) * (double)n;
                    }
                }
            }
        }
#pragma unroll
        for (int k = 0; k < P; ++k) {
            const int meta = st.meta[k];
            if (!(meta & BRM_VALID)) continue;
            const int kind = meta & 15;
            if (kind == SK_L) {
                double* zw = lds + Y.zl + buf * Y.NBT + st.zoff[k];
                zw[0] = st.z[k].x;
                zw[1] = st.z[k].y;
            } else if (kind < SK_GS) {
                const int raw = br_stage_raw<KIND>(kind), trn = br_stage_trn<KIND>(kind);
                double* dst = lds + BR_ST(Y, raw) + buf * Y.SU + st.zoff[k];
                if (meta & BRM_A0) dst[0] = st.z[k].x;
                if (meta & BRM_A1) dst[1] = st.z[k].y;
                if (trn >= 0) {
                    double* dw = lds + BR_ST(Y, trn) + buf * Y.SU + st.zoff[k];
                    if (meta & BRM_A0) dw[0] = st.lam[k].x;
                    if (meta & BRM_A1) dw[1] = st.lam[k].y;
                }
            } else {
                double* dst = lds + L.wk + M.K + (kind == SK_GLS ? M.nt1 : 0) + st.zoff[k];
                if (A.count_globals) {
                    if (meta & BRM_A0) dst[0] = st.z[k].x;
                    if (meta & BRM_A1) dst[1] = st.z[k].y;
                }
            }
        }
    }
    BB_STAMP_WAVE(cx, S, A, 0);
    BB_SYNC(cx);
    BB_STAMP(cx, S, 21);
}

#ifndef BB_EMU
template <int CTRL>
__device__ __forceinline__ double br_dpp(double x) {
    int lo = __double2loint(x), hi = __double2hiint(x);
    lo = __builtin_amdgcn_update_dpp(0, lo, CTRL, 0xF, 0xF, false);
    hi = __builtin_amdgcn_update_dpp(0, hi, CTRL, 0xF, 0xF, false);
    return __hiloint2double(hi, lo);
}
__device__ __forceinline__ double br_row16_sum(double s) {
    s += br_dpp<0x128>(s);
    s += br_dpp<0x124>(s);
    s += br_dpp<0x122>(s);
    s += br_dpp<0x121>(s);
    return s;
}
#endif

template <int P, bool MS = false>
BB_DEV void br_row_publish(BBCtx& cx, const DevModel& M, const DevState& S, const BRLay& Y, BRSt<P>* stv, unsigned epoch, bool want_el = false) {
    double* lds = cx.lds;
    BB_STAMP(cx, S, 23);
    const int KK = M.K + 2 * M.nt1, KS = bb_row_stride(KK);
    const int* rm = (const int*)(lds + Y.rowmap);
    const int nbt = ((const int*)(lds + Y.L.misc))[2];
    BB_PASS(cx, tid) {
        const int c = tid & 15;
        if (MS && tid == 0) {
            double e = 0.0;
            if (want_el) {
#ifdef BB_EMU
                if (stv) for (int t2 = 0; t2 < cx.nthr; ++t2) e += BB_PSTATE(stv, t2).el;
                else for (int w = 0; w < (cx.nthr + 63) / 64; ++w) e += lds[Y.L.part + w];
#else
                for (int w = 0; w < (cx.nthr >> 6); ++w) e += lds[Y.L.part + w];
#endif
            }
            lds[Y.L.wk + M.K - 2] = e;
        }
        for (int j = tid >> 4; j < M.K; j += cx.nthr >> 4) {
            if (MS && j == M.K - 2) continue;
            const int code = rm[2 * j], lpb = code & 255;
            const double* col = lds + rm[2 * j + 1];
            double s = 0.0;
#ifdef BB_EMU
            if (c == 0 && (code >> 24)) for (int e = 0; e < nbt; ++e) s += col[e * lpb];
#else
            if (code >> 24) for (int e = c; e < nbt; e += 16) s += col[e * lpb];
            s = br_row16_sum(s);
#endif
            if (c == 0) lds[Y.L.wk + j] = s;
        }
    }
    BB_SYNC(cx);
    int* li = (int*)(lds + Y.L.misc);
    BB_PASS(cx, tid) {
        if (li[4] > 0) { for (int j = tid; j < KK; j += cx.nthr) bb_gran_st_l2(S.grow + (long long)cx.block * KS + j, lds[Y.L.wk + j], epoch); }
        else for (int j = tid; j < KK; j += cx.nthr) bb_gran_st(S.grow + (long long)cx.block * KS + j, lds[Y.L.wk + j], epoch);
        if (tid == 0 && li[4] == 0) {
            int g = cx.block;
            while (g >= li[7]) g -= li[7];
            const unsigned long long v = bb_get_word64(S.xtab + g);
            if ((unsigned)(v >> 32) == (unsigned)li[6]) { li[4] = (int)(unsigned)v == li[5] ? 1 : -1; S.xsel[cx.block] = li[4]; }
        }
    }
    BB_STAMP(cx, S, 24);
    BB_STAMP_RT(cx, S, 29);
}

template <int KIND, int P, int TT> BB_DEV void br_theta_pre(BBCtx& cx, const DevModel& M, const BRLay& Y, BRSt<P>* stv, int buf);
template <int KIND, int P, bool MS = false>
BB_DEV void br_moments(BBCtx& cx, const DevModel& M, const DevState& S, const BRLay& Y, BRSt<P>* stv, int buf, unsigned epoch, bool want_el = false) {
    double* lds = cx.lds;
    if (KIND == 2) br_theta_pre<KIND, P, 0>(cx, M, Y, stv, buf);
    if (MS && want_el) {
        BB_PASS(cx, tid) {
            BRSt<P>& st = BB_PSTATE(stv, tid);
#ifdef BB_EMU
            (void)st;
#else
            double e = br_row16_sum(st.el);
            const int lo = __double2loint(e), hi = __double2hiint(e);
            double w = 0.0;
#pragma unroll
            for (int r = 0; r < 4; ++r) w += __hiloint2double(__builtin_amdgcn_readlane(hi, 16 * r), __builtin_amdgcn_readlane(lo, 16 * r));
            if ((tid & 63) == 0) lds[Y.L.part + (tid >> 6)] = w;
#endif
        }
    }
    BB_PASS(cx, tid) {
        BRSt<P>& st = BB_PSTATE(stv, tid);
#pragma unroll
        for (int k = 0; k < P; ++k) {
            const int meta = st.meta[k];
            if ((meta & 15) != SK_L) continue;
            double cv[BR_NCV];
#pragma unroll
            for (int q = 0; q < BR_NCV; ++q) cv[q] = 0.0;
            if (meta & BRM_VALID) {
            const double* zb = lds + Y.zl + buf * Y.NBT + st.zoff[k];
            const bool hn = meta & BRM_NEXT, mut = meta & BRM_MUT;
            const double z0 = st.z[k].x, z1 = st.z[k].y;
            const double zn = hn ? zb[2] : z1;
            double dm = z1 - z0, dn = zn - z1;
            cv[0] += st.lam[k].x;
            cv[6] += st.lam[k].y;
            if (mut) {
                double sm, sn, wm, wn;
                br_unit_sw<KIND>(lds, Y, buf, st.uo[k][1], KIND >= 2 ? st.thoff[k] : 0, &sm, &wm);
                if (KIND == 1 || KIND == 4) br_unit_sw<KIND>(lds, Y, buf, st.uo[k][2], KIND >= 3 ? st.thoff[k] : 0, &sn, &wn);
                else { sn = sm; wn = wm; }
                dm -= sm; dn -= sn;
                cv[1] += wm; cv[2] += wm * dm; cv[3] += wm * dm * dm;
                if (hn) { cv[7] += wn; cv[8] += wn * dn; cv[9] += wn * dn * dn; }
            } else {
                cv[4] += dm; cv[5] += dm * dm;
                if (hn) { cv[10] += dn; cv[11] += dn * dn; }
            }
            }
            {
                const BRSeg* sgk = (const BRSeg*)(lds + Y.seg) + (meta >> 12);
                const int stride = sgk->rstride;
#pragma unroll
                for (int q = 0; q < BR_NCV; ++q) lds[st.rb[k] + q * stride] = cv[q];
            }
        }
    }
    BB_SYNC(cx);
    br_row_publish<P, MS>(cx, M, S, Y, stv, epoch, want_el);
}

template <int P, bool HD>
BB_DEV void br_prefetch_slot(BBCtx& cx, const DevModel& M, const DevState& S, const RunArgs& A, const BRLay& Y, BRSt<P>* stv, int slot) {
    if (A.opt != 0) return;
    BB_PASS(cx, tid) {
        BRSt<P>& st = BB_PSTATE(stv, tid);
#pragma unroll
        for (int k = 0; k < P; ++k) {
            if (!(st.meta[k] & BRM_VALID)) continue;
#pragma unroll
            for (int which = 0; which < 2; ++which) {
                const double* src = S.hist + ((long long)slot * 2 + which) * M.Dh + (st.i0[k] - BR_HDELTA(HD, cx.lds, Y, st.meta[k]));
                bb_d2* dst = (bb_d2*)(cx.lds + Y.hbuf) + (k * 2 + which) * cx.nthr;
#ifdef BB_EMU
                dst[tid] = bb_d2{src[0], src[1]};
#else
                __builtin_amdgcn_global_load_lds((const __attribute__((address_space(1))) void*)src,
                                                 (__attribute__((address_space(3))) void*)(dst + (tid & ~63)), 16, 0, 0);
#endif
            }
        }
    }
}

template <int KIND, bool MS = false>
BB_DEV void br_finish(BBCtx& cx, const DevModel& M, const DevState& S, const BRLay& Y, const RunArgs* Ap = nullptr, bool want_el = false, int ring = 0, int smp = 0) {
    double* lds = cx.lds;
    const BBLds& L = Y.L;
    BB_STAMP(cx, S, 25);
    BB_STAMP_RT(cx, S, 30);
    BB_PASS(cx, tid) {
        for (int j = tid; j < M.Ttot; j += cx.nthr) {
            const int* ft = (const int*)(lds + Y.ftab) + 4 * j;
            const int mo = ft[0], zo = ft[1], hasprev = ft[2];
            double Dt = 0.0, c = 0.0, wb = 0.0;
            if (mo >= 0) {
                const double nn = (double)M.nn;
                const double* mm = lds + mo;
                const double M0 = mm[0], M1 = mm[1], N1 = mm[3], N2 = mm[4];
                const double sbar = lds[L.zgl + zo], ls = lds[L.zgl + M.nt1 + zo];
                wb = bb_exp(-2.0 * ls);
                c = lds[L.Lt + j + 1] - lds[L.Lt + j] - sbar;
                const double quadN = N2 - 2.0 * c * N1 + nn * c * c;
                Dt = (M1 - c * M0) + wb * (N1 - c * nn);
                lds[L.gglob + zo] = -Dt;
                lds[L.gglob + M.nt1 + zo] = wb * quadN - nn;
                if (MS && want_el) {
                    const double M2 = mm[2], quadM = M2 - 2.0 * c * M1 + c * c * M0;
                    lds[L.elbt + j] = -0.5 * (quadM + wb * quadN) - nn * ls;
                }
            } else if (MS && want_el) lds[L.elbt + j] = 0.0;
            lds[L.cc + j] = c;
            lds[L.wbar + j] = wb;
            lds[L.Dt + j] = Dt;
            lds[Y.iG + j] = ((hasprev ? lds[L.Dt + j - 1] : 0.0) - Dt) * lds[L.invS + j];
        }
    }
    BB_SYNC(cx);
    BB_STAMP(cx, S, 26);
    if (MS && want_el && cx.block == 0) {
        BB_PASS(cx, tid) {
            if (tid == 0) {
                const RunArgs& A = *Ap;
                double v = lds[L.wk + M.K - 2] + lds[L.wk + M.K - 1] + A.elbo_const;
                for (int j = 0; j < M.Ttot; ++j) v += lds[L.elbt + j];
                double* slot = S.elbo_ring + ring;
                *slot = (smp == 0 ? 0.0 : *slot) + v / (double)A.S;
            }
        }
    }
}

template <int KIND, int P>
BB_DEV void br_pair_prior(const double* lds, const BRLay& Y, const BRSt<P>& st, int k, bool a0, bool a1, double* pm0, double* iv0, double* pm1, double* iv1) {
    const BRSeg* sgk = (const BRSeg*)(lds + Y.seg) + (st.meta[k] >> 12);
    *pm0 = *pm1 = sgk->pm;
    *iv0 = *iv1 = sgk->iv;
    if (sgk->mean_e) {
        const long long j = st.i0[k] - sgk->blo;
        if (a0) { *pm0 = sgk->mean_e[j]; *iv0 = sgk->iv_e[j]; }
        if (a1) { *pm1 = sgk->mean_e[j + 1]; *iv1 = sgk->iv_e[j + 1]; }
    }
}
template <int KIND, int P>
BB_DEV void br_pair_diffs(const double* lds, const BRLay& Y, const BRSt<P>& st, int k, int buf, double* z0, double* z1,
                          double* ap, double* am, double* an, double* wp, double* wm, double* wn) {
    const int meta = st.meta[k];
    const bool hp = meta & BRM_PREV, hn = meta & BRM_NEXT;
    const double* zb = lds + Y.zl + buf * Y.NBT + st.zoff[k];
    *z0 = zb[0]; *z1 = zb[1];
    const double zp = hp ? zb[-1] : *z0, zn = hn ? zb[2] : *z1;
    *ap = *z0 - zp; *am = *z1 - *z0; *an = zn - *z1;
    *wp = *wm = *wn = 0.0;
    if (meta & BRM_MUT) {
        double sp, sm, sn;
        br_unit_sw<KIND>(lds, Y, buf, st.uo[k][1], KIND >= 2 ? st.thoff[k] : 0, &sm, wm);
        if (KIND == 1 || KIND == 4) {
            br_unit_sw<KIND>(lds, Y, buf, st.uo[k][0], KIND >= 3 ? st.thoff[k] : 0, &sp, wp);
            br_unit_sw<KIND>(lds, Y, buf, st.uo[k][2], KIND >= 3 ? st.thoff[k] : 0, &sn, wn);
        } else { sp = sn = sm; *wp = *wn = *wm; }
        *ap -= sp; *am -= sm; *an -= sn;
    }
}
template <int KIND, int P> BB_DEV constexpr bool br_has_pre() { return P == 1 && KIND <= 1; }
template <int KIND, int P, bool AP = false>
BB_DEV void br_grad_pre(BBCtx& cx, const BRLay& Y, BRSt<P>* stv, int buf) {
    if (!br_has_pre<KIND, P>()) return;
    const double* lds = cx.lds;
    BB_PASS(cx, tid) {
        BRSt<P>& st = BB_PSTATE(stv, tid);
#pragma unroll
        for (int k = 0; k < P; ++k) {
            const int meta = st.meta[k];
            if ((meta & 15) != SK_L || !(meta & BRM_VALID)) continue;
            const bool hp = meta & BRM_PREV, hn = meta & BRM_NEXT;
            double pm0, iv0, pm1, iv1, z0, z1, ap, am, an, wp, wm, wn;
            br_pair_prior<KIND>(lds, Y, st, k, true, AP ? (st.meta[k] & BRM_A1) != 0 : true, &pm0, &iv0, &pm1, &iv1);
            br_pair_diffs<KIND>(lds, Y, st, k, buf, &z0, &z1, &ap, &am, &an, &wp, &wm, &wn);
            double A0 = ((double)st.cnt[k][0] - st.lam[k].x) - (z0 - pm0) * iv0;
            double A1 = ((double)st.cnt[k][1] - st.lam[k].y) - (z1 - pm1) * iv1;
            if (meta & BRM_MUT) {
                const double ma = (AP && !(meta & BRM_A1)) ? 0.0 : wm * am;
                A0 += ma - (hp ? wp * ap : 0.0);
                A1 += (hn ? wn * an : 0.0) - ma;
            }
            st.gp[k] = bb_d2{A0, A1};
        }
    }
}
template <int KIND, int P, int TT>
BB_DEV void br_theta_pre(BBCtx& cx, const DevModel& M, const BRLay& Y, BRSt<P>* stv, int buf) {
    if (KIND != 2 && KIND != 3) return;
    double* lds = cx.lds;
    BB_PASS(cx, tid) {
        BRSt<P>& st = BB_PSTATE(stv, tid);
#pragma unroll
        for (int k = 0; k < P; ++k) {
            const int meta = st.meta[k];
            if ((meta & 15) != SK_TT_R || !(meta & BRM_VALID)) continue;
            const int* rt = (const int*)(lds + Y.rtab) + 4 * (KIND == 2 ? 0 : st.pt[k]);
            const int T = TT ? TT : rt[2];
            const double* zbuf = lds + Y.zl + buf * Y.NBT + (KIND == 2 ? Y.zr0[0] : rt[1]);
#pragma unroll
            for (int x = 0; x < 2; ++x) {
                if (!(meta & (x ? BRM_A1 : BRM_A0))) continue;
                const int j = st.zoff[k] + x, bl = st.uo[k][x];
                const int th = KIND == 2 ? j - ((st.uo[k][2] >> (16 * x)) & 0xffff) : st.thoff[k];
                double sv, wv;
                br_unit_sw<KIND>(lds, Y, buf, j, th, &sv, &wv);
                const double* zr = zbuf + bl * (T + 1);
                *(bb_d2*)(lds + Y.gas + 2 * j) = bb_d2{wv * ((zr[T - 1] - zr[0]) - (double)(T - 1) * sv), wv};
            }
        }
    }
}

template <int KIND, int P>
BB_DEV void br_theta_sum(BBCtx& cx, const DevModel& M, const BRLay& Y, BRSt<P>* stv) {
    if (KIND != 2) return;
    const double* lds = cx.lds;
    BB_PASS(cx, tid) {
        BRSt<P>& st = BB_PSTATE(stv, tid);
#pragma unroll
        for (int k = 0; k < P; ++k) {
            const int meta = st.meta[k];
            if ((meta & 15) != SK_TH_R || !(meta & BRM_VALID)) continue;
            bb_d2 sa{0.0, 0.0}, sw{0.0, 0.0};
#pragma unroll
            for (int x = 0; x < 2; ++x) {
                if (!(meta & (x ? BRM_A1 : BRM_A0))) continue;
                const int first = st.uo[k][x] & 0xffff, n = st.uo[k][x] >> 16;
                const bb_d2* ge = (const bb_d2*)(lds + Y.gas) + first;
                double a = 0.0, w = 0.0;
                int i = 0;
                for (; i + 4 <= n; i += 4) {
                    const bb_d2 e0 = ge[i], e1 = ge[i + 1], e2 = ge[i + 2], e3 = ge[i + 3];
                    a += (e0.x + e1.x) + (e2.x + e3.x);
                    w += (e0.y + e1.y) + (e2.y + e3.y);
                }
                for (; i < n; ++i) { a += ge[i].x; w += ge[i].y; }
                if (x) { sa.y = a; sw.y = w; } else { sa.x = a; sw.x = w; }
            }
            st.gp[k] = sa;
            st.lam[k] = sw;
        }
    }
}

template <int KIND, int P, bool AP = false, bool PRE = (P == 1 && KIND <= 1)>
BB_DEV void br_l_grad(const double* lds, const BRLay& Y, const BRSt<P>& st, int k, int buf, double* g0, double* g1) {
    const BBLds& L = Y.L;
    const int meta = st.meta[k], pt = st.pt[k];
    const bool hp = meta & BRM_PREV, hn = meta & BRM_NEXT;
    const double cp = hp ? lds[L.cc + pt - 1] : 0.0, cm = lds[L.cc + pt], cn = hn ? lds[L.cc + pt + 1] : 0.0;
    if (!PRE) {
        double pm0, iv0, pm1, iv1, z0, z1, ap, am, an, wp, wm, wn;
        br_pair_prior<KIND>(lds, Y, st, k, true, AP ? (st.meta[k] & BRM_A1) != 0 : true, &pm0, &iv0, &pm1, &iv1);
        br_pair_diffs<KIND>(lds, Y, st, k, buf, &z0, &z1, &ap, &am, &an, &wp, &wm, &wn);
        if (!(meta & BRM_MUT)) { wp = hp ? lds[L.wbar + pt - 1] : 0.0; wm = lds[L.wbar + pt]; wn = lds[L.wbar + pt + 1]; }
        const double rp_ = hp ? wp * (ap - cp) : 0.0, rm_ = (AP && !(meta & BRM_A1)) ? 0.0 : wm * (am - cm), rn_ = hn ? wn * (an - cn) : 0.0;
        const double l0 = st.lam[k].x, l1 = st.lam[k].y;
        *g0 = ((double)st.cnt[k][0] - l0) + l0 * lds[Y.iG + pt] + rm_ - rp_ - (z0 - pm0) * iv0;
        *g1 = ((double)st.cnt[k][1] - l1) + l1 * lds[Y.iG + pt + 1] + rn_ - rm_ - (z1 - pm1) * iv1;
        return;
    }
    double rp, rm, rn;
    if (meta & BRM_MUT) {
        double s_, wp, wm, wn;
        br_unit_sw<KIND>(lds, Y, buf, st.uo[k][1], KIND >= 2 ? st.thoff[k] : 0, &s_, &wm);
        if (KIND == 1 || KIND == 4) {
            br_unit_sw<KIND>(lds, Y, buf, st.uo[k][0], KIND >= 3 ? st.thoff[k] : 0, &s_, &wp);
            br_unit_sw<KIND>(lds, Y, buf, st.uo[k][2], KIND >= 3 ? st.thoff[k] : 0, &s_, &wn);
        } else { wp = wn = wm; }
        rp = -(wp * cp); rm = -(wm * cm); rn = -(wn * cn);
    } else {
        double z0, z1, ap, am, an, wp, wm, wn;
        br_pair_diffs<KIND>(lds, Y, st, k, buf, &z0, &z1, &ap, &am, &an, &wp, &wm, &wn);
        rp = hp ? lds[L.wbar + pt - 1] * (ap - cp) : 0.0;
        rm = (AP && !(meta & BRM_A1)) ? 0.0 : lds[L.wbar + pt] * (am - cm);
        rn = hn ? lds[L.wbar + pt + 1] * (an - cn) : 0.0;
    }
    *g0 = fma(st.lam[k].x, lds[Y.iG + pt], st.gp[k].x) + (rm - rp);
    *g1 = fma(st.lam[k].y, lds[Y.iG + pt + 1], st.gp[k].y) + (rn - rm);
}

template <int KIND, int P, int TT = 0, bool AP = false, bool MS = false, bool HD = false>
BB_DEV void br_update(BBCtx& cx, const DevModel& M, const DevState& S, const RunArgs& A, const BRLay& Y, BRSt<P>* stv,
                      const BBSlot wslot, int buf, int NBs, int smp = 0, int NS = 1) {
    double* lds = cx.lds;
    const BBLds& L = Y.L;
    BB_STAMP_WAVE(cx, S, A, 2);
#ifndef BB_EMU
    {
        bool u = false;
#pragma unroll
        for (int k = 0; k < P; ++k) u = u || ((stv->meta[k] & BRM_VALID) && (stv->meta[k] & 15) != SK_L);
        if (__builtin_amdgcn_ballot_w64(u) != 0ull) __builtin_amdgcn_s_setprio(3);
    }
#endif
    const double* zbuf = lds + Y.zl + buf * Y.NBT;
    BB_PASS(cx, tid) {
        BRSt<P>& st = BB_PSTATE(stv, tid);
        double* hs_m = nullptr;
        double* hs_o = nullptr;
        if (A.opt == 0) {
            hs_m = S.hist + ((long long)wslot.slot * 2 + 0) * M.Dh;
            hs_o = S.hist + ((long long)wslot.slot * 2 + 1) * M.Dh;
        }
#pragma unroll
        for (int k = 0; k < P; ++k) {
            const int meta = st.meta[k];
            if (!(meta & BRM_VALID)) continue;
            const int kind = meta & 15;
            const bool a0 = meta & BRM_A0, a1 = meta & BRM_A1;
            double pm0 = 0.0, pm1 = 0.0, iv0 = 0.0, iv1 = 0.0;
            if (kind != SK_L) br_pair_prior<KIND>(lds, Y, st, k, a0, a1, &pm0, &iv0, &pm1, &iv1);
            double g0 = 0.0, g1 = 0.0, z0 = 0.0, z1 = 0.0;
            if (kind == SK_L) {
                br_l_grad<KIND, P, AP>(lds, Y, st, k, buf, &g0, &g1);
            } else if (KIND == 2 && kind == SK_TH_R) {
                const double* stg = lds + buf * Y.SU;
                double csum = 0.0;
                { const int T = TT ? TT : M.T[0]; for (int tt = 0; tt < T - 1; ++tt) csum += lds[L.cc + tt]; }
#pragma unroll
                for (int x = 0; x < 2; ++x) {
                    if (!(x ? a1 : a0)) continue;
                    (x ? g1 : g0) = (x ? st.gp[k].y : st.gp[k].x) - (x ? st.lam[k].y : st.lam[k].x) * csum;
                    (x ? z1 : z0) = stg[BR_ST(Y, 3) + st.zoff[k] + x];
                }
            } else if (kind < SK_GS) {
                const int* envt = (const int*)(lds + Y.envt);
                const double* stg = lds + buf * Y.SU;
                const int E = (KIND == 1 || KIND == 4) ? M.E : 1;
                double gx[2] = {0.0, 0.0}, zx[2] = {0.0, 0.0};
#pragma unroll
                for (int x = 0; x < 2; ++x) {
                    if (!(x ? a1 : a0)) continue;
                    const int j = st.zoff[k] + x;
                    const int e = KIND == 2 ? 0 : (st.uo[k][2] >> (8 * x)) & 255, bl = st.uo[k][x];
                    zx[x] = stg[BR_ST(Y, br_stage_raw<KIND>(kind)) + j];
                    const bool is_th = KIND >= 3 && kind == SK_TH_R;
                    if (KIND == 3 && is_th) {
                        double acc = 0.0;
                        for (int r = 0; r < M.R; ++r) {
                            const int* rt = (const int*)(lds + Y.rtab) + 4 * r;
                            const int T = TT ? TT : rt[2];
                            double csum = 0.0;
                            for (int tt = 0; tt < T - 1; ++tt) csum += lds[L.cc + rt[0] + tt];
                            const bb_d2 ge = *(const bb_d2*)(lds + Y.gas + 2 * (r * NBs + j));
                            acc += ge.x - ge.y * csum;
                        }
                        gx[x] = acc;
                        continue;
                    }
                    const int r0 = KIND <= 1 ? 0 : (is_th ? 0 : st.pt[k]), r1 = KIND <= 1 ? 1 : (is_th ? M.R : r0 + 1);
                    double acc = 0.0;
                    for (int r = r0; r < r1; ++r) {
                        const int o = is_th ? (r * NBs + (j / E)) * E + e : j;
                        const int th = KIND <= 1 ? 0 : (KIND == 2 ? j - ((st.uo[k][2] >> (16 * x)) & 0xffff) : (is_th ? r * NBs * E : st.thoff[k]));
                        double sv, wv;
                        br_unit_sw<KIND>(lds, Y, buf, o, th, &sv, &wv);
                        const int* rt = (const int*)(lds + Y.rtab) + 4 * r;
                        const int T = TT ? TT : rt[2], tc = KIND <= 1 ? 0 : rt[0];
                        const double* zr = zbuf + (KIND <= 1 ? Y.zr0[0] : rt[1]) + bl * (T + 1);
                        double As = 0.0, Qs = 0.0;
                        int nn = 0;
                        if (TT) {
                            double zrow[TT ? TT : 1];
#pragma unroll
                            for (int tt = 0; tt < TT; ++tt) zrow[tt] = zr[tt];
#pragma unroll
                            for (int tt = 0; tt < TT - 1; ++tt) {
                                const bool use = E == 1 || envt[tc + tt + 1] == e;
                                const double rr = use ? (zrow[tt + 1] - zrow[tt]) - sv - lds[L.cc + tc + tt] : 0.0;
                                As += rr; Qs += rr * rr; nn += use ? 1 : 0;
                            }
                        } else {
                            for (int tt = 0; tt < T - 1; ++tt) {
                                if (E > 1 && envt[tc + tt + 1] != e) continue;
                                const double rr = (zr[tt + 1] - zr[tt]) - sv - lds[L.cc + tc + tt];
                                As += rr; Qs += rr * rr; ++nn;
                            }
                        }
                        if (KIND <= 1) acc = kind == SK_S ? wv * As : wv * Qs - (double)nn;
                        else if (is_th) acc += wv * As;
                        else if (kind == SK_LS_R) acc = wv * Qs - (double)nn;
                        else if (kind == SK_TT_R) acc = wv * As * stg[BR_ST(Y, 1) + j];
                        else acc = wv * As * stg[BR_ST(Y, 1) + j] * stg[BR_ST(Y, 0) + j];
                    }
                    gx[x] = acc;
                }
                g0 = gx[0]; g1 = gx[1]; z0 = zx[0]; z1 = zx[1];
            } else {
                const double* gg = lds + L.gglob + (kind == SK_GLS ? M.nt1 : 0) + st.zoff[k];
                const double* zz = lds + L.zgl + (kind == SK_GLS ? M.nt1 : 0) + st.zoff[k];
                if (a0) { g0 = gg[0]; z0 = zz[0]; }
                if (a1) { g1 = gg[1]; z1 = zz[1]; }
            }
            g0 -= (z0 - pm0) * iv0;
            g1 -= (z1 - pm1) * iv1;
            double go0, go1;
            if (MS && NS > 1) {
                go0 = g0 * st.a[k].x; go1 = g1 * st.a[k].y;
                if (smp > 0) { g0 += st.gm[k].x; g1 += st.gm[k].y; go0 += st.go[k].x; go1 += st.go[k].y; }
                if (smp < NS - 1) { st.gm[k] = bb_d2{g0, g1}; st.go[k] = bb_d2{go0, go1}; continue; }
                const double invS = 1.0 / (double)NS;
                g0 *= invS; g1 *= invS;
                go0 = go0 * invS + st.h[k].x; go1 = go1 * invS + st.h[k].y;
            } else { go0 = fma(g0, st.a[k].x, st.h[k].x); go1 = fma(g1, st.a[k].y, st.h[k].y); }
            bb_d2 hm{0, 0}, ho{0, 0};
            if (hs_m) {
#ifndef BB_EMU
                asm volatile("s_waitcnt vmcnt(0)" ::: "memory");
#endif
                hm = ((const bb_d2*)(lds + Y.hbuf))[(k * 2 + 0) * cx.nthr + tid];
                ho = ((const bb_d2*)(lds + Y.hbuf))[(k * 2 + 1) * cx.nthr + tid];
            }
            bb_d2 nhm = hm, nho = ho;
            const long long ih = st.i0[k] - BR_HDELTA(HD, lds, Y, meta);
            if (a0) {
                bb_opt_apply(M, S, A, wslot, 0, ih, -g0, hm.x, &nhm.x, &st.mu[k].x, &st.am[k].x, &st.lo[k].x);
                BR_SCHED_FENCE();
                bb_opt_apply(M, S, A, wslot, 1, ih, -go0, ho.x, &nho.x, &st.om[k].x, &st.ao[k].x, &st.lo[k].y);
                BR_SCHED_FENCE();
            }
            if (a1) {
                bb_opt_apply(M, S, A, wslot, 0, ih + 1, -g1, hm.y, &nhm.y, &st.mu[k].y, &st.am[k].y, &st.lo[k].z);
                BR_SCHED_FENCE();
                bb_opt_apply(M, S, A, wslot, 1, ih + 1, -go1, ho.y, &nho.y, &st.om[k].y, &st.ao[k].y, &st.lo[k].w);
                BR_SCHED_FENCE();
            }
            if (hs_m) { br_store_pair_stream<AP>(hs_m, ih, a0, a1, nhm); br_store_pair_stream<AP>(hs_o, ih, a0, a1, nho); }
        }
    }
#ifndef BB_EMU
    __builtin_amdgcn_s_setprio(0);
#endif
    BB_STAMP_WAVE(cx, S, A, 3);
    BB_STAMP(cx, S, 28);
}

template <int KIND, int P, bool AP = false>
BB_DEV void br_epilogue(BBCtx& cx, const DevState& S, BRSt<P>* stv, unsigned long long step_end, bool timed_out) {
    BB_PASS(cx, tid) {
        BRSt<P>& st = BB_PSTATE(stv, tid);
        bool bad = false;
#pragma unroll
        for (int k = 0; k < P; ++k) {
            const int meta = st.meta[k];
            if (!(meta & BRM_VALID)) continue;
            const bool a0 = meta & BRM_A0, a1 = meta & BRM_A1;
            br_store_pair<AP>(S.mu, st.i0[k], a0, a1, st.mu[k]);
            br_store_pair<AP>(S.om, st.i0[k], a0, a1, st.om[k]);
            br_store_pair<AP>(S.acc_mu, st.i0[k], a0, a1, st.am[k]);
            br_store_pair<AP>(S.acc_om, st.i0[k], a0, a1, st.ao[k]);
            bb_store_lo(S, st.i0[k], a0, a1, st.lo[k]);
            const double chk = (a0 ? st.mu[k].x + st.om[k].x : 0.0) + (a1 ? st.mu[k].y + st.om[k].y : 0.0);
            bad = bad || !(chk - chk == 0.0);
        }
        if (bad) S.hstatus[1] = 1u;
        if (timed_out && tid == 0) S.hstatus[0] = 1u;
        if (cx.block == 0 && tid == 0) { S.ctr[0] = step_end; S.ctr[1] = step_end; }
    }
    BB_SYNC(cx);
}

template <int KIND, int P, bool AP = false, bool HD = false>
BB_DEV void br_xchg_publish(BBCtx& cx, const DevModel& M, const DevState& S, const RunArgs& A, const BRLay& Y, BRSt<P>* stv, unsigned long long xc, int slot,
                            unsigned long long next_step, unsigned next_stream = 0u, bool prefetch = true) {
    if (A.pf == 0 && prefetch) br_prefetch_slot<P, HD>(cx, M, S, A, Y, stv, slot);
    br_grad_pre<KIND, P, AP>(cx, Y, stv, (int)(xc & 1));
    br_theta_sum<KIND, P>(cx, M, Y, stv);
    if (KIND == 3) br_theta_pre<KIND, P, 0>(cx, M, Y, stv, (int)(xc & 1));
    br_draw_ahead<KIND, P, AP>(cx, A, Y, stv, next_step, next_stream);
}
template <bool XG>
BB_DEV void br_xchg_lead(BBCtx& cx, const DevModel& M, const DevState& S, const RunArgs& A, const BRLay& Y, unsigned long long xc, int* ok_slot) {
    const unsigned epoch = A.xepoch0 + (unsigned)(xc + 1);
    if (cx.block < bbp_groups(A)) bbp_leader_reduce_tg<XG>(cx, M, S, A, Y.L, (int)(xc & 1), epoch, ok_slot);
}
template <int KIND, int P, bool XG, bool MS = false>
BB_DEV void br_xchg_consume(BBCtx& cx, const DevModel& M, const DevState& S, const RunArgs& A, const BRLay& Y, BRSt<P>* stv,
                            unsigned long long xc, int* ok_slot, bool want_el = false, int ring = 0, int smp = 0) {
    const unsigned epoch = A.xepoch0 + (unsigned)(xc + 1);
    if (XG) bbp_consume_tgx(cx, M, S, A, Y.L, (int)(xc & 1), epoch, ok_slot);
    else bbp_consume_tg(cx, M, S, A, Y.L, (int)(xc & 1), epoch, ok_slot);
    br_finish<KIND, MS>(cx, M, S, Y, &A, want_el, ring, smp);
}

#ifndef BB_EMU
template <int KIND, int P, int NT, bool XG = false, int TT = 0, bool AP = false, bool MS = false>
__global__ void __launch_bounds__(NT) k_res(const DevModel* __restrict__ Mp, const DevState* __restrict__ Sp, const BRLay* __restrict__ Yp,
                                            RunArgs A, int NB, int nsteps) {
    const DevModel& M = *Mp;
    const DevState& S = *Sp;
    const BRLay& Y = *Yp;
    extern __shared__ __attribute__((aligned(16))) double br_smem[];
    BBCtx cx{(int)blockDim.x, (int)blockIdx.x, br_smem, nullptr};
    BRSt<P> st;
    int* ok_slot = (int*)(br_smem + Yp->L.misc) + 1;
    const unsigned long long c0 = S.ctr[0], c1 = S.ctr[1];
    unsigned long long step0 = c0 > c1 ? c0 : c1;
    step0 = ((unsigned long long)(unsigned)__builtin_amdgcn_readfirstlane((int)(step0 >> 32)) << 32) | (unsigned)__builtin_amdgcn_readfirstlane((int)step0);
    BB_STAMP_RT(cx, S, 2);
    br_prologue<KIND, P, AP>(cx, M, S, A, Y, NB, &st);
    BB_STAMP_RT(cx, S, 3);
    const bool dead = *ok_slot == 0;
    int done = 0;
    if (!dead) {
        br_draw_ahead<KIND, P, AP>(cx, A, Y, &st, step0);
        BB_STAMP_RT(cx, S, 4);
        BBSlotCtr sc = bb_slot_init(A, step0);
        const int NS = MS ? A.S : 1;
        int ec = (MS && A.elbo_every > 0) ? bb_uniform((int)(step0 % (unsigned long long)A.elbo_every)) : 1;
        int ring = (MS && A.elbo_every > 0) ? bb_uniform((int)(((step0 + (unsigned long long)A.elbo_every - 1ull) / (unsigned long long)A.elbo_every) % BB_ELBO_RING)) : 0;
        for (; done < nsteps; ++done, bb_slot_next(A, sc)) {
            const unsigned long long step = step0 + (unsigned long long)done;
            const BBSlot wslot = bb_slot_now(A, sc);
            const bool want_el = MS && A.elbo_every > 0 && ec == 0;
            bool stop = false;
            for (int smp = 0; smp < NS; ++smp) {
                const unsigned long long xc = MS ? step * (unsigned long long)NS + (unsigned long long)smp : step;
                const int buf = (int)(xc & 1);
                const bool last = smp == NS - 1;
                if (P > 1 || KIND >= 2) {
#pragma unroll
                    for (int k = 0; k < P; ++k) asm volatile("" : "+v"(st.meta[k]));
                }
                br_sample<KIND, P, MS, XG>(cx, M, S, A, Y, &st, buf, wslot.slot, last, want_el);
                br_moments<KIND, P, MS>(cx, M, S, Y, &st, buf, A.xepoch0 + (unsigned)(xc + 1), want_el);
                br_xchg_publish<KIND, P, AP, XG>(cx, M, S, A, Y, &st, xc, wslot.slot, last ? step + 1 : step, last ? 0u : (unsigned)(smp + 1), last);
                br_xchg_lead<XG>(cx, M, S, A, Y, xc, ok_slot);
                br_xchg_consume<KIND, P, XG, MS>(cx, M, S, A, Y, &st, xc, ok_slot, want_el, ring, smp);
                if (*ok_slot == 0) { stop = true; break; }
                br_update<KIND, P, TT, AP, MS, XG>(cx, M, S, A, Y, &st, wslot, buf, NB, smp, NS);
            }
            if (stop) break;
            if (MS && A.elbo_every > 0) {
                if (ec == 0) ring = ring + 1 == BB_ELBO_RING ? 0 : ring + 1;
                ec = ec + 1 == A.elbo_every ? 0 : ec + 1;
            }
        }
    }
    BB_STAMP_RT(cx, S, 5);
    asm volatile("s_waitcnt vmcnt(0)" ::: "memory");
    br_epilogue<KIND, P, AP>(cx, S, &st, step0 + (unsigned long long)done, dead || *ok_slot == 0);
    BB_STAMP_RT(cx, S, 6);
}
#endif
```

barbay.jl_amd/csrc/bb_types.h:

```cpp
#pragma once
#include <stdint.h>

#define BB_MAX_REP 16

enum BBBlockKind {
    BK_SPOP = 0,
    BK_LSPOP = 1,
    BK_S = 2,
    BK_TT = 3,
    BK_LT = 4,
    BK_LS = 5,
    BK_L = 6,
    BK_COUNT = 7
};

#define BB_NQ 6

struct DevPrior {
    double mean, inv_var;
    const double* mean_e;
    const double* inv_var_e;
};

struct DevModel {
    int kind, R, E, G;
    long long nn, nb, B, D;
    long long Dp;
    long long Dh;
    long long hd0[BK_COUNT], hd1[BK_COUNT];
    long long hdl[BB_MAX_REP];
    int T[BB_MAX_REP];
    unsigned Tmagic[BB_MAX_REP];
    unsigned Tmagic1[BB_MAX_REP];
    long long off_l[BB_MAX_REP];
    int off_t[BB_MAX_REP];
    long long cnt_off[BB_MAX_REP];
    int kq[BB_MAX_REP];
    int kqa[BB_MAX_REP];
    int quirk;
    int tcum[BB_MAX_REP];
    int Ttot, nt1, K;
    long long blk_lo[BK_COUNT], blk_hi[BK_COUNT];
    DevPrior pri[BK_COUNT];
    const int* env_idx;
    const int* geno_idx;
    const int* geno_ptr;
    const int* geno_mem;
    int geno_sorted;
    const unsigned* counts;
    const double* piv;
};

#define BB_MAX_WORLD 16

struct bb_gran;
struct DevState {
    double *mu, *om;
    double *zsv, *asv, *hsv;
    double *acc_mu, *acc_om;
    double *hist;
    const double *optc;
    float *accl;
    double *gacc_mu, *gacc_om;
    double *partials;
    double *totals;
    double *zg;
    double *ztheta;
    double *ds;
    double *gsum;
    double *geno_el;
    double *elbo_ring;
    double *elbo_sample;
    unsigned long long *ctr;
    const double *eps_in;
    unsigned *gbar;
    unsigned *hstatus;
    double *prow;
    double *xrow;
    struct bb_gran *grow, *gxrow;
    unsigned *rdy;
    int *xsel;
    unsigned long long *xtab;
    const double *segtab;
    int segtab_stride;
    const int *ldstab;
    const long long *tile_b;
    const int *tile_g;
    unsigned long long *stamps;
    double *xout[BB_MAX_WORLD];
    unsigned *xout_rdy[BB_MAX_WORLD];
    struct bb_gran *xgr[BB_MAX_WORLD];
};

#define BB_ELBO_RING 4096

struct RunArgs {
    long long b_lo, b_hi;
    int rank, world;
    unsigned xepoch0;
    unsigned spin_limit;
    unsigned launch_tag;
    int row_l2;
    int nblk;
    int nblk_alloc;
    int ng;
    int pf;
    int nbl;
    int par;
    int sample, S;
    int first_sample, last_sample;
    int apply;
    int with_elbo;
    int count_globals;
    int opt, W, resum_every, elbo_every;
    double eta, tau, pre, post;
    unsigned long long seed;
    const double* red;
    int nred;
    double elbo_const;
};
```

Measured before the change: 71960.

## Specialize resident-kernel sample/grad/update paths per wave-uniform parameter role

At tile setup, each wave checks by ballot whether all its lanes hold the same parameter kind (L, S, or LS-env) and stores that uniform role. The sample, grad-pre and update stages then dispatch to role-templated thread functions, so branches on the per-lane kind become compile-time constants and dead paths are dropped. Sample also saves softplus and defers the reciprocal for h to a separate pass after the exchange, taking it off the critical sampling path. The cost is more code size and register state per thread (role plus an sp array). An env knob can turn the roles off.

```diff
diff --git a/barbay.jl_amd/csrc/bb_engine.hip b/barbay.jl_amd/csrc/bb_engine.hip
--- a/barbay.jl_amd/csrc/bb_engine.hip
+++ b/barbay.jl_amd/csrc/bb_engine.hip
@@ -42,7 +42,7 @@
 struct BBTuning {
     bool no_hist_pack, no_host_tables, no_res, no_persist, no_stream, force_stream, any_parity, force_allreduce, p2p_self;
     bool no_graph, graph_collective, no_regroup, no_reorder, nb_set, lead_set;
-    int nb, res_nb, ng, lead, nthr, row_l2;
+    int nb, res_nb, ng, lead, nthr, row_l2, no_roles;
 };
 
 static BBTuning read_tuning() {
@@ -72,6 +72,7 @@
     if (t.lead < 10 || t.lead > 100) t.lead = 100;
     t.nthr = num("BB_TUNE_NTHR", 0) >= 64 ? num("BB_TUNE_NTHR", 0) / 64 * 64 : 0;
     t.row_l2 = num("BB_TUNE_ROW_L2", 1) == 0 ? 0 : 1;
+    t.no_roles = on("BB_TUNE_NO_ROLES") ? 1 : 0;
     return t;
 }
 
@@ -1345,6 +1346,7 @@
     A.xepoch0 = h->epoch0;
     A.spin_limit = 1u << 23;
     A.row_l2 = h->tune.row_l2;
+    A.no_roles = h->tune.no_roles;
     A.nblk = h->nblk;
     A.nblk_alloc = h->tile_cap - 8;
     A.ng = 8;
diff --git a/barbay.jl_amd/csrc/bb_resident.h b/barbay.jl_amd/csrc/bb_resident.h
--- a/barbay.jl_amd/csrc/bb_resident.h
+++ b/barbay.jl_amd/csrc/bb_resident.h
@@ -179,9 +179,61 @@
     bb_d2 gp[P];
     bb_d2 gm[P], go[P];
     double el;
+    int role;
+    bb_d2 sp[P];
 };
 
 enum { BRM_A0 = 1 << 4, BRM_A1 = 1 << 5, BRM_VALID = 1 << 6, BRM_MUT = 1 << 7, BRM_PREV = 1 << 8, BRM_NEXT = 1 << 9 };
+
+enum { BRR_GEN = 0, BRR_L = 1, BRR_S = 2, BRR_LS = 3 };
+template <int KIND, int P> BB_DEV constexpr bool br_has_roles() {
+#ifdef BR_NO_ROLES
+    return false;
+#else
+    return P == 1 && KIND <= 1;
+#endif
+}
+template <int KIND, int P> BB_DEV constexpr bool br_late_h() {
+#ifdef BR_NO_LATE_H
+    return false;
+#else
+    return P == 1 && KIND <= 1;
+#endif
+}
+#ifdef BB_EMU
+#define BR_OPAQUE(x) ((void)0)
+#else
+#define BR_OPAQUE(x) asm volatile("" : "+v"(x))
+#endif
+template <int ROLE> BB_DEV int br_role_meta(int meta) {
+    const int full = BRM_A0 | BRM_A1 | BRM_VALID;
+    if (ROLE == BRR_L) return (meta & ~(15 | full)) | SK_L | full;
+    if (ROLE == BRR_S) return (meta & ~0xfff) | SK_S | full;
+    if (ROLE == BRR_LS) return (meta & ~0xfff) | SK_LS_E | full;
+    return meta;
+}
+template <int P>
+BB_DEV int br_wave_role(const BBCtx& cx, const RunArgs& A, BRSt<P>* stv, int tid) {
+    const int full = BRM_A0 | BRM_A1 | BRM_VALID, mask = 15 | full;
+    int role = BRR_GEN;
+#ifdef BB_EMU
+    const int w0 = tid & ~63;
+    if (w0 + 64 <= cx.nthr) {
+        const int key = stv[w0].meta[0] & mask;
+        bool same = true;
+        for (int t2 = w0; t2 < w0 + 64; ++t2) same = same && (stv[t2].meta[0] & mask) == key;
+        if (same) role = key == (SK_L | full) ? BRR_L : (key == (SK_S | full) ? BRR_S : (key == (SK_LS_E | full) ? BRR_LS : BRR_GEN));
+    }
+    return A.no_roles ? BRR_GEN : role;
+#else
+    (void)cx; (void)tid;
+    const int key = stv->meta[0] & mask;
+    if (__builtin_amdgcn_ballot_w64(key != (SK_L | full)) == 0ull) role = BRR_L;
+    else if (__builtin_amdgcn_ballot_w64(key != (SK_S | full)) == 0ull) role = BRR_S;
+    else if (__builtin_amdgcn_ballot_w64(key != (SK_LS_E | full)) == 0ull) role = BRR_LS;
+    return __builtin_amdgcn_readfirstlane(A.no_roles ? BRR_GEN : role);
+#endif
+}
 
 template <bool AP> BB_DEV bool br_pair_aligned(long long i0) { return !AP || !(i0 & 1); }
 template <bool AP> BB_DEV bb_d2 br_load_pair(const double* base, long long i0, bool a0, bool a1) {
@@ -483,6 +535,9 @@
             st.a[k] = st.h[k] = st.z[k] = st.lam[k] = st.gp[k] = bb_d2{0.0, 0.0};
         }
     }
+    if (br_has_roles<KIND, P>()) {
+        BB_PASS(cx, tid) { BB_PSTATE(stv, tid).role = br_wave_role<P>(cx, A, stv, tid); }
+    }
     BB_STAMP_RT(cx, S, 10);
     BB_SYNC(cx);
 }
@@ -551,100 +606,110 @@
 template <int P, bool HD = false>
 BB_DEV void br_prefetch_slot(BBCtx& cx, const DevModel& M, const DevState& S, const RunArgs& A, const BRLay& Y, BRSt<P>* stv, int slot);
 template <int KIND, int P> BB_DEV void br_pair_prior(const double* lds, const BRLay& Y, const BRSt<P>& st, int k, bool a0, bool a1, double* pm0, double* iv0, double* pm1, double* iv1);
+template <int KIND, int P, bool MS, int ROLE>
+BB_DEV void br_sample_thread(BBCtx& cx, const DevModel& M, const RunArgs& A, const BRLay& Y, BRSt<P>& st, int tid, int buf, bool want_el) {
+    double* lds = cx.lds;
+    const BBLds& L = Y.L;
+#pragma unroll
+    for (int k = 0; k < P; ++k) {
+        const int meta_k = br_role_meta<ROLE>(st.meta[k]);
+#ifdef BB_EMU
+        if (!(meta_k & BRM_VALID)) continue;
+#else
+        if (P > 1 && __builtin_amdgcn_ballot_w64((meta_k & BRM_VALID) != 0) == 0ull) continue;
+#endif
+        const bb_d2 e = ((const bb_d2*)(lds + Y.eps))[k * cx.nthr + tid];
+        double sp0, sg0, sp1, sg1;
+        bb_softplus_sigmoid(st.om[k].x, &sp0, &sg0);
+        bb_softplus_sigmoid(st.om[k].y, &sp1, &sg1);
+        st.z[k] = bb_d2{fma(sp0, e.x, st.mu[k].x), fma(sp1, e.y, st.mu[k].y)};
+        st.a[k] = bb_d2{e.x * sg0, e.y * sg1};
+        if (br_late_h<KIND, P>()) { st.sp[k] = bb_d2{sp0, sp1}; st.h[k] = bb_d2{sg0, sg1}; }
+        else st.h[k] = bb_d2{sg0 * bb_rcp(sp0), sg1 * bb_rcp(sp1)};
+        if (MS && want_el) {
+            if (k == 0) st.el = 0.0;
+            const int meta = meta_k, kd = meta & 15;
+            const bool counted = (meta & BRM_VALID) && (kd < SK_GS || A.count_globals);
+            if (counted) {
+                const bool a0 = meta & BRM_A0, a1 = meta & BRM_A1;
+                double pm0, iv0, pm1, iv1;
+                br_pair_prior<KIND>(lds, Y, st, k, a0, a1, &pm0, &iv0, &pm1, &iv1);
+                if (a0) st.el += -0.5 * (st.z[k].x - pm0) * (st.z[k].x - pm0) * iv0 + bb_log(sp0);
+                if (a1) st.el += -0.5 * (st.z[k].y - pm1) * (st.z[k].y - pm1) * iv1 + bb_log(sp1);
+            }
+        }
+        BR_SCHED_FENCE();
+        const int kd = meta_k & 15;
+        const double f = (kd == SK_LS_E || (KIND >= 2 && kd == SK_LS_R)) ? -2.0 : 1.0;
+#ifndef BB_EMU
+        if (ROLE == BRR_S || (ROLE == BRR_GEN && __builtin_amdgcn_ballot_w64((meta_k & BRM_VALID) && (kd == SK_L || (kd < SK_GS && br_stage_trn<KIND>(kd) >= 0))) == 0ull)) st.lam[k] = bb_d2{0.0, 0.0};
+        else
+#endif
+        st.lam[k] = bb_d2{bb_exp(f * st.z[k].x), bb_exp(f * st.z[k].y)};
+        BR_SCHED_FENCE();
+        if (MS && want_el && (meta_k & BRM_VALID)) {
+            const int meta = meta_k;
+            if (kd == SK_L) {
+                st.el += (double)st.cnt[k][0] * st.z[k].x - st.lam[k].x;
+                if (meta & BRM_A1) st.el += (double)st.cnt[k][1] * st.z[k].y - st.lam[k].y;
+            } else if (kd == SK_LS_E || (KIND >= 2 && kd == SK_LS_R)) {
+                const BRSeg* sgk = (const BRSeg*)(lds + Y.seg) + (meta >> 12);
+                const int T1 = sgk->T - 1;
+#pragma unroll
+                for (int x = 0; x < 2; ++x) {
+                    if (!(meta & (x ? BRM_A1 : BRM_A0))) continue;
+                    int n = T1;
+                    if (KIND == 1 || KIND == 4) {
+                        const int* envt = (const int*)(lds + Y.envt);
+                        const int e_ = (st.uo[k][2] >> (8 * x)) & 255, tc = KIND == 4 ? M.tcum[st.pt[k]] : 0;
+                        n = 0;
+                        for (int tt = 0; tt < T1; ++tt) n += envt[tc + tt + 1] == e_ ? 1 : 0;
+                    }
+                    st.el -= (x ? st.z[k].y : st.z[k].x) * (double)n;
+                }
+            }
+        }
+    }
+#pragma unroll
+    for (int k = 0; k < P; ++k) {
+        const int meta = br_role_meta<ROLE>(st.meta[k]);
+        if (!(meta & BRM_VALID)) continue;
+        const int kind = meta & 15;
+        if (kind == SK_L) {
+            double* zw = lds + Y.zl + buf * Y.NBT + st.zoff[k];
+            zw[0] = st.z[k].x;
+            zw[1] = st.z[k].y;
+        } else if (kind < SK_GS) {
+            const int raw = br_stage_raw<KIND>(kind), trn = br_stage_trn<KIND>(kind);
+            double* dst = lds + BR_ST(Y, raw) + buf * Y.SU + st.zoff[k];
+            if (meta & BRM_A0) dst[0] = st.z[k].x;
+            if (meta & BRM_A1) dst[1] = st.z[k].y;
+            if (trn >= 0) {
+                double* dw = lds + BR_ST(Y, trn) + buf * Y.SU + st.zoff[k];
+                if (meta & BRM_A0) dw[0] = st.lam[k].x;
+                if (meta & BRM_A1) dw[1] = st.lam[k].y;
+            }
+        } else {
+            double* dst = lds + L.wk + M.K + (kind == SK_GLS ? M.nt1 : 0) + st.zoff[k];
+            if (A.count_globals) {
+                if (meta & BRM_A0) dst[0] = st.z[k].x;
+                if (meta & BRM_A1) dst[1] = st.z[k].y;
+            }
+        }
+    }
+}
 template <int KIND, int P, bool MS = false, bool HD = false>
 BB_DEV void br_sample(BBCtx& cx, const DevModel& M, const DevState& S, const RunArgs& A, const BRLay& Y, BRSt<P>* stv, int buf, int slot, bool prefetch = true, bool want_el = false) {
-    double* lds = cx.lds;
-    const BBLds& L = Y.L;
     BB_STAMP(cx, S, 20);
     BB_STAMP_WAVE(cx, S, A, 1);
     if (A.pf == 1 && prefetch) br_prefetch_slot<P, HD>(cx, M, S, A, Y, stv, slot);
     BB_PASS(cx, tid) {
         BRSt<P>& st = BB_PSTATE(stv, tid);
-#pragma unroll
-        for (int k = 0; k < P; ++k) {
-#ifdef BB_EMU
-            if (!(st.meta[k] & BRM_VALID)) continue;
-#else
-            if (P > 1 && __builtin_amdgcn_ballot_w64((st.meta[k] & BRM_VALID) != 0) == 0ull) continue;
-#endif
-            const bb_d2 e = ((const bb_d2*)(lds + Y.eps))[k * cx.nthr + tid];
-            double sp0, sg0, sp1, sg1;
-            bb_softplus_sigmoid(st.om[k].x, &sp0, &sg0);
-            bb_softplus_sigmoid(st.om[k].y, &sp1, &sg1);
-            st.z[k] = bb_d2{fma(sp0, e.x, st.mu[k].x), fma(sp1, e.y, st.mu[k].y)};
-            st.a[k] = bb_d2{e.x * sg0, e.y * sg1};
-            st.h[k] = bb_d2{sg0 * bb_rcp(sp0), sg1 * bb_rcp(sp1)};
-            if (MS && want_el) {
-                if (k == 0) st.el = 0.0;
-                const int meta = st.meta[k], kd = meta & 15;
-                const bool counted = (meta & BRM_VALID) && (kd < SK_GS || A.count_globals);
-                if (counted) {
-                    const bool a0 = meta & BRM_A0, a1 = meta & BRM_A1;
-                    double pm0, iv0, pm1, iv1;
-                    br_pair_prior<KIND>(lds, Y, st, k, a0, a1, &pm0, &iv0, &pm1, &iv1);
-                    if (a0) st.el += -0.5 * (st.z[k].x - pm0) * (st.z[k].x - pm0) * iv0 + bb_log(sp0);
-                    if (a1) st.el += -0.5 * (st.z[k].y - pm1) * (st.z[k].y - pm1) * iv1 + bb_log(sp1);
-                }
-            }
-            BR_SCHED_FENCE();
-            const int kd = st.meta[k] & 15;
-            const double f = (kd == SK_LS_E || (KIND >= 2 && kd == SK_LS_R)) ? -2.0 : 1.0;
-#ifndef BB_EMU
-            if (__builtin_amdgcn_ballot_w64((st.meta[k] & BRM_VALID) && (kd == SK_L || (kd < SK_GS && br_stage_trn<KIND>(kd) >= 0))) == 0ull) st.lam[k] = bb_d2{0.0, 0.0};
-            else
-#endif
-            st.lam[k] = bb_d2{bb_exp(f * st.z[k].x), bb_exp(f * st.z[k].y)};
-            BR_SCHED_FENCE();
-            if (MS && want_el && (st.meta[k] & BRM_VALID)) {
-                const int meta = st.meta[k];
-                if (kd == SK_L) {
-                    st.el += (double)st.cnt[k][0] * st.z[k].x - st.lam[k].x;
-                    if (meta & BRM_A1) st.el += (double)st.cnt[k][1] * st.z[k].y - st.lam[k].y;
-                } else if (kd == SK_LS_E || (KIND >= 2 && kd == SK_LS_R)) {
-                    const BRSeg* sgk = (const BRSeg*)(lds + Y.seg) + (meta >> 12);
-                    const int T1 = sgk->T - 1;
-#pragma unroll
-                    for (int x = 0; x < 2; ++x) {
-                        if (!(meta & (x ? BRM_A1 : BRM_A0))) continue;
-                        int n = T1;
-                        if (KIND == 1 || KIND == 4) {
-                            const int* envt = (const int*)(lds + Y.envt);
-                            const int e_ = (st.uo[k][2] >> (8 * x)) & 255, tc = KIND == 4 ? M.tcum[st.pt[k]] : 0;
-                            n = 0;
-                            for (int tt = 0; tt < T1; ++tt) n += envt[tc + tt + 1] == e_ ? 1 : 0;
-                        }
-                        st.el -= (x ? st.z[k].y : st.z[k].x) * (double)n;
-                    }
-                }
-            }
-        }
-#pragma unroll
-        for (int k = 0; k < P; ++k) {
-            const int meta = st.meta[k];
-            if (!(meta & BRM_VALID)) continue;
-            const int kind = meta & 15;
-            if (kind == SK_L) {
-                double* zw = lds + Y.zl + buf * Y.NBT + st.zoff[k];
-                zw[0] = st.z[k].x;
-                zw[1] = st.z[k].y;
-            } else if (kind < SK_GS) {
-                const int raw = br_stage_raw<KIND>(kind), trn = br_stage_trn<KIND>(kind);
-                double* dst = lds + BR_ST(Y, raw) + buf * Y.SU + st.zoff[k];
-                if (meta & BRM_A0) dst[0] = st.z[k].x;
-                if (meta & BRM_A1) dst[1] = st.z[k].y;
-                if (trn >= 0) {
-                    double* dw = lds + BR_ST(Y, trn) + buf * Y.SU + st.zoff[k];
-                    if (meta & BRM_A0) dw[0] = st.lam[k].x;
-                    if (meta & BRM_A1) dw[1] = st.lam[k].y;
-                }
-            } else {
-                double* dst = lds + L.wk + M.K + (kind == SK_GLS ? M.nt1 : 0) + st.zoff[k];
-                if (A.count_globals) {
-                    if (meta & BRM_A0) dst[0] = st.z[k].x;
-                    if (meta & BRM_A1) dst[1] = st.z[k].y;
-                }
-            }
-        }
+        const int role = br_has_roles<KIND, P>() ? st.role : BRR_GEN;
+        if (role == BRR_L) br_sample_thread<KIND, P, MS, BRR_L>(cx, M, A, Y, st, tid, buf, want_el);
+        else if (role == BRR_S) br_sample_thread<KIND, P, MS, BRR_S>(cx, M, A, Y, st, tid, buf, want_el);
+        else if (role == BRR_LS) br_sample_thread<KIND, P, MS, BRR_LS>(cx, M, A, Y, st, tid, buf, want_el);
+        else br_sample_thread<KIND, P, MS, BRR_GEN>(cx, M, A, Y, st, tid, buf, want_el);
     }
     BB_STAMP_WAVE(cx, S, A, 0);
     BB_SYNC(cx);
@@ -884,29 +949,44 @@
     }
 }
 template <int KIND, int P> BB_DEV constexpr bool br_has_pre() { return P == 1 && KIND <= 1; }
+template <int KIND, int P, bool AP, int ROLE>
+BB_DEV void br_grad_pre_thread(const double* lds, const BRLay& Y, BRSt<P>& st, int buf) {
+#pragma unroll
+    for (int k = 0; k < P; ++k) {
+        const int meta = br_role_meta<ROLE>(st.meta[k]);
+        if ((meta & 15) != SK_L || !(meta & BRM_VALID)) continue;
+        const bool hp = meta & BRM_PREV, hn = meta & BRM_NEXT;
+        double pm0, iv0, pm1, iv1, z0, z1, ap, am, an, wp, wm, wn;
+        br_pair_prior<KIND>(lds, Y, st, k, true, AP ? (meta & BRM_A1) != 0 : true, &pm0, &iv0, &pm1, &iv1);
+        br_pair_diffs<KIND>(lds, Y, st, k, buf, &z0, &z1, &ap, &am, &an, &wp, &wm, &wn);
+        double A0 = ((double)st.cnt[k][0] - st.lam[k].x) - (z0 - pm0) * iv0;
+        double A1 = ((double)st.cnt[k][1] - st.lam[k].y) - (z1 - pm1) * iv1;
+        if (meta & BRM_MUT) {
+            const double ma = (AP && !(meta & BRM_A1)) ? 0.0 : wm * am;
+            A0 += ma - (hp ? wp * ap : 0.0);
+            A1 += (hn ? wn * an : 0.0) - ma;
+        }
+        st.gp[k] = bb_d2{A0, A1};
+    }
+}
 template <int KIND, int P, bool AP = false>
 BB_DEV void br_grad_pre(BBCtx& cx, const BRLay& Y, BRSt<P>* stv, int buf) {
     if (!br_has_pre<KIND, P>()) return;
     const double* lds = cx.lds;
     BB_PASS(cx, tid) {
         BRSt<P>& st = BB_PSTATE(stv, tid);
-#pragma unroll
-        for (int k = 0; k < P; ++k) {
-            const int meta = st.meta[k];
-            if ((meta & 15) != SK_L || !(meta & BRM_VALID)) continue;
-            const bool hp = meta & BRM_PREV, hn = meta & BRM_NEXT;
-            double pm0, iv0, pm1, iv1, z0, z1, ap, am, an, wp, wm, wn;
-            br_pair_prior<KIND>(lds, Y, st, k, true, AP ? (st.meta[k] & BRM_A1) != 0 : true, &pm0, &iv0, &pm1, &iv1);
-            br_pair_diffs<KIND>(lds, Y, st, k, buf, &z0, &z1, &ap, &am, &an, &wp, &wm, &wn);
-            double A0 = ((double)st.cnt[k][0] - st.lam[k].x) - (z0 - pm0) * iv0;
-            double A1 = ((double)st.cnt[k][1] - st.lam[k].y) - (z1 - pm1) * iv1;
-            if (meta & BRM_MUT) {
-                const double ma = (AP && !(meta & BRM_A1)) ? 0.0 : wm * am;
-                A0 += ma - (hp ? wp * ap : 0.0);
-                A1 += (hn ? wn * an : 0.0) - ma;
-            }
-            st.gp[k] = bb_d2{A0, A1};
-        }
+        const int role = br_has_roles<KIND, P>() ? st.role : BRR_GEN;
+        if (role == BRR_L) br_grad_pre_thread<KIND, P, AP, BRR_L>(lds, Y, st, buf);
+        else if (role == BRR_GEN) br_grad_pre_thread<KIND, P, AP, BRR_GEN>(lds, Y, st, buf);
+    }
+}
+template <int KIND, int P>
+BB_DEV void br_h_form(BBCtx& cx, BRSt<P>* stv) {
+    if (!br_late_h<KIND, P>()) return;
+    BB_PASS(cx, tid) {
+        BRSt<P>& st = BB_PSTATE(stv, tid);
+#pragma unroll
+        for (int k = 0; k < P; ++k) st.h[k] = bb_d2{st.h[k].x * bb_rcp(st.sp[k].x), st.h[k].y * bb_rcp(st.sp[k].y)};
     }
 }
 template <int KIND, int P, int TT>
@@ -1005,11 +1085,149 @@
     *g1 = fma(st.lam[k].y, lds[Y.iG + pt + 1], st.gp[k].y) + (rn - rm);
 }
 
+template <int KIND, int P, int TT, bool AP, bool MS, bool HD, int ROLE>
+BB_DEV void br_update_thread(BBCtx& cx, const DevModel& M, const DevState& S, const RunArgs& A, const BRLay& Y, BRSt<P>& st, int tid,
+                             const BBSlot wslot, int buf, int NBs, int smp, int NS) {
+    double* lds = cx.lds;
+    const BBLds& L = Y.L;
+    const double* zbuf = lds + Y.zl + buf * Y.NBT;
+    double* hs_m = nullptr;
+    double* hs_o = nullptr;
+    if (A.opt == 0) {
+        hs_m = S.hist + ((long long)wslot.slot * 2 + 0) * M.Dh;
+        hs_o = S.hist + ((long long)wslot.slot * 2 + 1) * M.Dh;
+    }
+#pragma unroll
+    for (int k = 0; k < P; ++k) {
+        const int meta = br_role_meta<ROLE>(st.meta[k]);
+        if (!(meta & BRM_VALID)) continue;
+        const int kind = meta & 15;
+        const bool a0 = meta & BRM_A0, a1 = meta & BRM_A1;
+        double pm0 = 0.0, pm1 = 0.0, iv0 = 0.0, iv1 = 0.0;
+        if (kind != SK_L) br_pair_prior<KIND>(lds, Y, st, k, a0, a1, &pm0, &iv0, &pm1, &iv1);
+        double g0 = 0.0, g1 = 0.0, z0 = 0.0, z1 = 0.0;
+        if (kind == SK_L) {
+            br_l_grad<KIND, P, AP>(lds, Y, st, k, buf, &g0, &g1);
+        } else if (KIND == 2 && kind == SK_TH_R) {
+            const double* stg = lds + buf * Y.SU;
+            double csum = 0.0;
+            { const int T = TT ? TT : M.T[0]; for (int tt = 0; tt < T - 1; ++tt) csum += lds[L.cc + tt]; }
+#pragma unroll
+            for (int x = 0; x < 2; ++x) {
+                if (!(x ? a1 : a0)) continue;
+                (x ? g1 : g0) = (x ? st.gp[k].y : st.gp[k].x) - (x ? st.lam[k].y : st.lam[k].x) * csum;
+                (x ? z1 : z0) = stg[BR_ST(Y, 3) + st.zoff[k] + x];
+            }
+        } else if (kind < SK_GS) {
+            const int* envt = (const int*)(lds + Y.envt);
+            const double* stg = lds + buf * Y.SU;
+            const int E = (KIND == 1 || KIND == 4) ? M.E : 1;
+            double gx[2] = {0.0, 0.0}, zx[2] = {0.0, 0.0};
+#pragma unroll
+            for (int x = 0; x < 2; ++x) {
+                if (!(x ? a1 : a0)) continue;
+                const int j = st.zoff[k] + x;
+                const int e = KIND == 2 ? 0 : (st.uo[k][2] >> (8 * x)) & 255, bl = st.uo[k][x];
+                zx[x] = stg[BR_ST(Y, br_stage_raw<KIND>(kind)) + j];
+                const bool is_th = KIND >= 3 && kind == SK_TH_R;
+                if (KIND == 3 && is_th) {
+                    double acc = 0.0;
+                    for (int r = 0; r < M.R; ++r) {
+                        const int* rt = (const int*)(lds + Y.rtab) + 4 * r;
+                        const int T = TT ? TT : rt[2];
+                        double csum = 0.0;
+                        for (int tt = 0; tt < T - 1; ++tt) csum += lds[L.cc + rt[0] + tt];
+                        const bb_d2 ge = *(const bb_d2*)(lds + Y.gas + 2 * (r * NBs + j));
+                        acc += ge.x - ge.y * csum;
+                    }
+                    gx[x] = acc;
+                    continue;
+                }
+                const int r0 = KIND <= 1 ? 0 : (is_th ? 0 : st.pt[k]), r1 = KIND <= 1 ? 1 : (is_th ? M.R : r0 + 1);
+                double acc = 0.0;
+                for (int r = r0; r < r1; ++r) {
+                    const int o = is_th ? (r * NBs + (j / E)) * E + e : j;
+                    const int th = KIND <= 1 ? 0 : (KIND == 2 ? j - ((st.uo[k][2] >> (16 * x)) & 0xffff) : (is_th ? r * NBs * E : st.thoff[k]));
+                    double sv, wv;
+                    br_unit_sw<KIND>(lds, Y, buf, o, th, &sv, &wv);
+                    const int* rt = (const int*)(lds + Y.rtab) + 4 * r;
+                    const int T = TT ? TT : rt[2], tc = KIND <= 1 ? 0 : rt[0];
+                    const double* zr = zbuf + (KIND <= 1 ? Y.zr0[0] : rt[1]) + bl * (T + 1);
+                    double As = 0.0, Qs = 0.0;
+                    int nn = 0;
+                    if (TT) {
+                        double zrow[TT ? TT : 1];
+#pragma unroll
+                        for (int tt = 0; tt < TT; ++tt) zrow[tt] = zr[tt];
+#pragma unroll
+                        for (int tt = 0; tt < TT - 1; ++tt) {
+                            const bool use = E == 1 || envt[tc + tt + 1] == e;
+                            const double rr = use ? (zrow[tt + 1] - zrow[tt]) - sv - lds[L.cc + tc + tt] : 0.0;
+                            As += rr; Qs += rr * rr; nn += use ? 1 : 0;
+                        }
+                    } else {
+                        for (int tt = 0; tt < T - 1; ++tt) {
+                            if (E > 1 && envt[tc + tt + 1] != e) continue;
+                            const double rr = (zr[tt + 1] - zr[tt]) - sv - lds[L.cc + tc + tt];
+                            As += rr; Qs += rr * rr; ++nn;
+                        }
+                    }
+                    if (KIND <= 1) acc = kind == SK_S ? wv * As : wv * Qs - (double)nn;
+                    else if (is_th) acc += wv * As;
+                    else if (kind == SK_LS_R) acc = wv * Qs - (double)nn;
+                    else if (kind == SK_TT_R) acc = wv * As * stg[BR_ST(Y, 1) + j];
+                    else acc = wv * As * stg[BR_ST(Y, 1) + j] * stg[BR_ST(Y, 0) + j];
+                }
+                gx[x] = acc;
+            }
+            g0 = gx[0]; g1 = gx[1]; z0 = zx[0]; z1 = zx[1];
+        } else {
+            const double* gg = lds + L.gglob + (kind == SK_GLS ? M.nt1 : 0) + st.zoff[k];
+            const double* zz = lds + L.zgl + (kind == SK_GLS ? M.nt1 : 0) + st.zoff[k];
+            if (a0) { g0 = gg[0]; z0 = zz[0]; }
+            if (a1) { g1 = gg[1]; z1 = zz[1]; }
+        }
+        if (ROLE != BRR_GEN) { BR_OPAQUE(g0); BR_OPAQUE(g1); }
+        g0 -= (z0 - pm0) * iv0;
+        g1 -= (z1 - pm1) * iv1;
+        double go0, go1;
+        if (MS && NS > 1) {
+            go0 = g0 * st.a[k].x; go1 = g1 * st.a[k].y;
+            if (smp > 0) { g0 += st.gm[k].x; g1 += st.gm[k].y; go0 += st.go[k].x; go1 += st.go[k].y; }
+            if (smp < NS - 1) { st.gm[k] = bb_d2{g0, g1}; st.go[k] = bb_d2{go0, go1}; continue; }
+            const double invS = 1.0 / (double)NS;
+            g0 *= invS; g1 *= invS;
+            go0 = go0 * invS + st.h[k].x; go1 = go1 * invS + st.h[k].y;
+        } else { go0 = fma(g0, st.a[k].x, st.h[k].x); go1 = fma(g1, st.a[k].y, st.h[k].y); }
+        bb_d2 hm{0, 0}, ho{0, 0};
+        if (hs_m) {
+#ifndef BB_EMU
+            asm volatile("s_waitcnt vmcnt(0)" ::: "memory");
+#endif
+            hm = ((const bb_d2*)(lds + Y.hbuf))[(k * 2 + 0) * cx.nthr + tid];
+            ho = ((const bb_d2*)(lds + Y.hbuf))[(k * 2 + 1) * cx.nthr + tid];
+        }
+        bb_d2 nhm = hm, nho = ho;
+        const long long ih = st.i0[k] - BR_HDELTA(HD, lds, Y, meta);
+        if (a0) {
+            bb_opt_apply(M, S, A, wslot, 0, ih, -g0, hm.x, &nhm.x, &st.mu[k].x, &st.am[k].x, &st.lo[k].x);
+            BR_SCHED_FENCE();
+            bb_opt_apply(M, S, A, wslot, 1, ih, -go0, ho.x, &nho.x, &st.om[k].x, &st.ao[k].x, &st.lo[k].y);
+            BR_SCHED_FENCE();
+        }
+        if (a1) {
+            bb_opt_apply(M, S, A, wslot, 0, ih + 1, -g1, hm.y, &nhm.y, &st.mu[k].y, &st.am[k].y, &st.lo[k].z);
+            BR_SCHED_FENCE();
+            bb_opt_apply(M, S, A, wslot, 1, ih + 1, -go1, ho.y, &nho.y, &st.om[k].y, &st.ao[k].y, &st.lo[k].w);
+            BR_SCHED_FENCE();
+        }
+        if (hs_m) { br_store_pair_stream<AP>(hs_m, ih, a0, a1, nhm); br_store_pair_stream<AP>(hs_o, ih, a0, a1, nho); }
+    }
+}
+
 template <int KIND, int P, int TT = 0, bool AP = false, bool MS = false, bool HD = false>
 BB_DEV void br_update(BBCtx& cx, const DevModel& M, const DevState& S, const RunArgs& A, const BRLay& Y, BRSt<P>* stv,
                       const BBSlot wslot, int buf, int NBs, int smp = 0, int NS = 1) {
-    double* lds = cx.lds;
-    const BBLds& L = Y.L;
     BB_STAMP_WAVE(cx, S, A, 2);
 #ifndef BB_EMU
     {
@@ -1019,140 +1237,13 @@
         if (__builtin_amdgcn_ballot_w64(u) != 0ull) __builtin_amdgcn_s_setprio(3);
     }
 #endif
-    const double* zbuf = lds + Y.zl + buf * Y.NBT;
     BB_PASS(cx, tid) {
         BRSt<P>& st = BB_PSTATE(stv, tid);
-        double* hs_m = nullptr;
-        double* hs_o = nullptr;
-        if (A.opt == 0) {
-            hs_m = S.hist + ((long long)wslot.slot * 2 + 0) * M.Dh;
-            hs_o = S.hist + ((long long)wslot.slot * 2 + 1) * M.Dh;
-        }
-#pragma unroll
-        for (int k = 0; k < P; ++k) {
-            const int meta = st.meta[k];
-            if (!(meta & BRM_VALID)) continue;
-            const int kind = meta & 15;
-            const bool a0 = meta & BRM_A0, a1 = meta & BRM_A1;
-            double pm0 = 0.0, pm1 = 0.0, iv0 = 0.0, iv1 = 0.0;
-            if (kind != SK_L) br_pair_prior<KIND>(lds, Y, st, k, a0, a1, &pm0, &iv0, &pm1, &iv1);
-            double g0 = 0.0, g1 = 0.0, z0 = 0.0, z1 = 0.0;
-            if (kind == SK_L) {
-                br_l_grad<KIND, P, AP>(lds, Y, st, k, buf, &g0, &g1);
-            } else if (KIND == 2 && kind == SK_TH_R) {
-                const double* stg = lds + buf * Y.SU;
-                double csum = 0.0;
-                { const int T = TT ? TT : M.T[0]; for (int tt = 0; tt < T - 1; ++tt) csum += lds[L.cc + tt]; }
-#pragma unroll
-                for (int x = 0; x < 2; ++x) {
-                    if (!(x ? a1 : a0)) continue;
-                    (x ? g1 : g0) = (x ? st.gp[k].y : st.gp[k].x) - (x ? st.lam[k].y : st.lam[k].x) * csum;
-                    (x ? z1 : z0) = stg[BR_ST(Y, 3) + st.zoff[k] + x];
-                }
-            } else if (kind < SK_GS) {
-                const int* envt = (const int*)(lds + Y.envt);
-                const double* stg = lds + buf * Y.SU;
-                const int E = (KIND == 1 || KIND == 4) ? M.E : 1;
-                double gx[2] = {0.0, 0.0}, zx[2] = {0.0, 0.0};
-#pragma unroll
-                for (int x = 0; x < 2; ++x) {
-                    if (!(x ? a1 : a0)) continue;
-                    const int j = st.zoff[k] + x;
-                    const int e = KIND == 2 ? 0 : (st.uo[k][2] >> (8 * x)) & 255, bl = st.uo[k][x];
-                    zx[x] = stg[BR_ST(Y, br_stage_raw<KIND>(kind)) + j];
-                    const bool is_th = KIND >= 3 && kind == SK_TH_R;
-                    if (KIND == 3 && is_th) {
-                        double acc = 0.0;
-                        for (int r = 0; r < M.R; ++r) {
-                            const int* rt = (const int*)(lds + Y.rtab) + 4 * r;
-                            const int T = TT ? TT : rt[2];
-                            double csum = 0.0;
-                            for (int tt = 0; tt < T - 1; ++tt) csum += lds[L.cc + rt[0] + tt];
-                            const bb_d2 ge = *(const bb_d2*)(lds + Y.gas + 2 * (r * NBs + j));
-                            acc += ge.x - ge.y * csum;
-                        }
-                        gx[x] = acc;
-                        continue;
-                    }
-                    const int r0 = KIND <= 1 ? 0 : (is_th ? 0 : st.pt[k]), r1 = KIND <= 1 ? 1 : (is_th ? M.R : r0 + 1);
-                    double acc = 0.0;
-                    for (int r = r0; r < r1; ++r) {
-                        const int o = is_th ? (r * NBs + (j / E)) * E + e : j;
-                        const int th = KIND <= 1 ? 0 : (KIND == 2 ? j - ((st.uo[k][2] >> (16 * x)) & 0xffff) : (is_th ? r * NBs * E : st.thoff[k]));
-                        double sv, wv;
-                        br_unit_sw<KIND>(lds, Y, buf, o, th, &sv, &wv);
-                        const int* rt = (const int*)(lds + Y.rtab) + 4 * r;
-                        const int T = TT ? TT : rt[2], tc = KIND <= 1 ? 0 : rt[0];
-                        const double* zr = zbuf + (KIND <= 1 ? Y.zr0[0] : rt[1]) + bl * (T + 1);
-                        double As = 0.0, Qs = 0.0;
-                        int nn = 0;
-                        if (TT) {
-                            double zrow[TT ? TT : 1];
-#pragma unroll
-                            for (int tt = 0; tt < TT; ++tt) zrow[tt] = zr[tt];
-#pragma unroll
-                            for (int tt = 0; tt < TT - 1; ++tt) {
-                                const bool use = E == 1 || envt[tc + tt + 1] == e;
-                                const double rr = use ? (zrow[tt + 1] - zrow[tt]) - sv - lds[L.cc + tc + tt] : 0.0;
-                                As += rr; Qs += rr * rr; nn += use ? 1 : 0;
-                            }
-                        } else {
-                            for (int tt = 0; tt < T - 1; ++tt) {
-                                if (E > 1 && envt[tc + tt + 1] != e) continue;
-                                const double rr = (zr[tt + 1] - zr[tt]) - sv - lds[L.cc + tc + tt];
-                                As += rr; Qs += rr * rr; ++nn;
-                            }
-                        }
-                        if (KIND <= 1) acc = kind == SK_S ? wv * As : wv * Qs - (double)nn;
-                        else if (is_th) acc += wv * As;
-                        else if (kind == SK_LS_R) acc = wv * Qs - (double)nn;
-                        else if (kind == SK_TT_R) acc = wv * As * stg[BR_ST(Y, 1) + j];
-                        else acc = wv * As * stg[BR_ST(Y, 1) + j] * stg[BR_ST(Y, 0) + j];
-                    }
-                    gx[x] = acc;
-                }
-                g0 = gx[0]; g1 = gx[1]; z0 = zx[0]; z1 = zx[1];
-            } else {
-                const double* gg = lds + L.gglob + (kind == SK_GLS ? M.nt1 : 0) + st.zoff[k];
-                const double* zz = lds + L.zgl + (kind == SK_GLS ? M.nt1 : 0) + st.zoff[k];
-                if (a0) { g0 = gg[0]; z0 = zz[0]; }
-                if (a1) { g1 = gg[1]; z1 = zz[1]; }
-            }
-            g0 -= (z0 - pm0) * iv0;
-            g1 -= (z1 - pm1) * iv1;
-            double go0, go1;
-            if (MS && NS > 1) {
-                go0 = g0 * st.a[k].x; go1 = g1 * st.a[k].y;
-                if (smp > 0) { g0 += st.gm[k].x; g1 += st.gm[k].y; go0 += st.go[k].x; go1 += st.go[k].y; }
-                if (smp < NS - 1) { st.gm[k] = bb_d2{g0, g1}; st.go[k] = bb_d2{go0, go1}; continue; }
-                const double invS = 1.0 / (double)NS;
-                g0 *= invS; g1 *= invS;
-                go0 = go0 * invS + st.h[k].x; go1 = go1 * invS + st.h[k].y;
-            } else { go0 = fma(g0, st.a[k].x, st.h[k].x); go1 = fma(g1, st.a[k].y, st.h[k].y); }
-            bb_d2 hm{0, 0}, ho{0, 0};
-            if (hs_m) {
-#ifndef BB_EMU
-                asm volatile("s_waitcnt vmcnt(0)" ::: "memory");
-#endif
-                hm = ((const bb_d2*)(lds + Y.hbuf))[(k * 2 + 0) * cx.nthr + tid];
-                ho = ((const bb_d2*)(lds + Y.hbuf))[(k * 2 + 1) * cx.nthr + tid];
-            }
-            bb_d2 nhm = hm, nho = ho;
-            const long long ih = st.i0[k] - BR_HDELTA(HD, lds, Y, meta);
-            if (a0) {
-                bb_opt_apply(M, S, A, wslot, 0, ih, -g0, hm.x, &nhm.x, &st.mu[k].x, &st.am[k].x, &st.lo[k].x);
-                BR_SCHED_FENCE();
-                bb_opt_apply(M, S, A, wslot, 1, ih, -go0, ho.x, &nho.x, &st.om[k].x, &st.ao[k].x, &st.lo[k].y);
-                BR_SCHED_FENCE();
-            }
-            if (a1) {
-                bb_opt_apply(M, S, A, wslot, 0, ih + 1, -g1, hm.y, &nhm.y, &st.mu[k].y, &st.am[k].y, &st.lo[k].z);
-                BR_SCHED_FENCE();
-                bb_opt_apply(M, S, A, wslot, 1, ih + 1, -go1, ho.y, &nho.y, &st.om[k].y, &st.ao[k].y, &st.lo[k].w);
-                BR_SCHED_FENCE();
-            }
-            if (hs_m) { br_store_pair_stream<AP>(hs_m, ih, a0, a1, nhm); br_store_pair_stream<AP>(hs_o, ih, a0, a1, nho); }
-        }
+        const int role = br_has_roles<KIND, P>() ? st.role : BRR_GEN;
+        if (role == BRR_L) br_update_thread<KIND, P, TT, AP, MS, HD, BRR_L>(cx, M, S, A, Y, st, tid, wslot, buf, NBs, smp, NS);
+        else if (role == BRR_S) br_update_thread<KIND, P, TT, AP, MS, HD, BRR_S>(cx, M, S, A, Y, st, tid, wslot, buf, NBs, smp, NS);
+        else if (role == BRR_LS) br_update_thread<KIND, P, TT, AP, MS, HD, BRR_LS>(cx, M, S, A, Y, st, tid, wslot, buf, NBs, smp, NS);
+        else br_update_thread<KIND, P, TT, AP, MS, HD, BRR_GEN>(cx, M, S, A, Y, st, tid, wslot, buf, NBs, smp, NS);
     }
 #ifndef BB_EMU
     __builtin_amdgcn_s_setprio(0);
@@ -1191,6 +1282,7 @@
                             unsigned long long next_step, unsigned next_stream = 0u, bool prefetch = true) {
     if (A.pf == 0 && prefetch) br_prefetch_slot<P, HD>(cx, M, S, A, Y, stv, slot);
     br_grad_pre<KIND, P, AP>(cx, Y, stv, (int)(xc & 1));
+    br_h_form<KIND, P>(cx, stv);
     br_theta_sum<KIND, P>(cx, M, Y, stv);
     if (KIND == 3) br_theta_pre<KIND, P, 0>(cx, M, Y, stv, (int)(xc & 1));
     br_draw_ahead<KIND, P, AP>(cx, A, Y, stv, next_step, next_stream);
diff --git a/barbay.jl_amd/csrc/bb_types.h b/barbay.jl_amd/csrc/bb_types.h
--- a/barbay.jl_amd/csrc/bb_types.h
+++ b/barbay.jl_amd/csrc/bb_types.h
@@ -117,5 +117,6 @@
     unsigned long long seed;
     const double* red;
     int nred;
+    int no_roles;
     double elbo_const;
 };
```

Measured after the change: 72560 (median of 3 runs). No clear change (+0.8%).
